# lucidrains/transfusion-pytorch

Measured on NVIDIA H100. Metric: train tokens/sec (text+latent) at d=512 L=8 seq=1024, higher is better.
Workload: dtype bf16

## Files before the change

include/tfx_b200.h:

```cpp
#ifndef TFX_B200_H
#define TFX_B200_H

#ifdef __cplusplus
extern "C" {
#endif

#define TFX_B200_VERSION 200

const char* tfx_last_error(void);
int tfx_version(void);
int tfx_init(int device);


int tfx_gemm_set_cluster_mode(int mode);

int tfx_gemm_store(const void* A, long long lda, int a_mn_major, const void* B, long long ldb, int b_mn_major, int M, int N, int K,
                   float* out_f32, long long ld_f32, void* out_bf16, long long ld_bf16, const float* bias, const long long* row_off,
                   float alpha, int accumulate, int k_splits, void* stream);

int tfx_gemm_qkvg(const void* u, long long ldu, const void* W, long long ldw, int M, int H, int D, void* q, void* k, void* v, float* gates, float* qk_inv,
                  const float* q_gamma, const float* k_gamma, const int* rope_pos, const float* rope_cs_t , int rope_len,
                  const int* kv_rows, float* mix_pre, void* stream);

int tfx_gemm_resid(const void* A, long long lda, const void* A2, long long lda2, int K1, const void* W, long long ldw, int M, int N, int K, const float* bias,
                   const float* x_res, float* x_out, void* x_out_bf16, void* y_bf16, const int* cond_row, const float* zgate, long long zgate_ld,
                   const float* layerscale, void* stream);

int tfx_gemm_geglu(const void* u, long long ldu, const void* W1p, long long ldw, const float* b1p, int M, int Np, int K, void* vg, void* h, void* stream);
int tfx_gemm_geglu_drop(const void* u, long long ldu, const void* W1p, long long ldw, const float* b1p, int M, int Np, int K, void* vg, void* h,
                        const void* drop_key , float p, int layer, void* stream);

int tfx_attn_fwd(const void* q, const void* k, const void* v, long long ld_q, long long ld_k, long long ld_v, const float* gates, int H,
                 const int* kv_limit, const int* tile_q0, const int* tile_qend, const int* tile_kv0, const int* tile_kvend, int n_tiles,
                 void* o, long long ld_o, float* lse, int M, float scale, float softcap, const float* skip_if_fast , void* stream);
int tfx_attn_fast_params(const float* q_gamma, const float* k_gamma, int dim_head, float scale, float softcap, float* params , void* stream);
int tfx_attn_fwd_tc(const void* q, const void* k, const void* v, long long ld_q, long long ld_k, long long ld_v, const float* gates, int H,
                    const int* kv_limit, const int* tile_q0, const int* tile_qend, const int* tile_kv0, const int* tile_kvend, int n_tiles,
                    void* o, long long ld_o, float* lse, int M, int M_kv , float scale, float softcap,
                    const float* fast_params, void* stream);
int tfx_attn_bwd_prep(const void* do_gated, const void* o_gated, const float* gates, void* do_pre, float* dsum_hm, float* dsum_mh, float* dq_zero, int M, int H, void* stream);
int tfx_attn_bwd(const void* q, const void* k, const void* v, const void* do_pre, long long ld_q, long long ld_k, long long ld_v, long long ld_do,
                 const float* lse, const float* dsum_hm, const int* kv_limit, const int* kt_kv0, const int* kt_kvend, const int* kt_q0, const int* kt_qend,
                 int n_kv_tiles, float* dq, float* dk, void* dv, long long ld_dv, int M, int H, float scale, float softcap, const float* skip_if_fast ,
                 void* stream);
int tfx_attn_bwd_tc(const void* q, const void* k, const void* v, const void* do_pre, long long ld_q, long long ld_k, long long ld_v, long long ld_do,
                    const float* lse, const float* dsum_hm, const int* kv_limit, const int* kt_kv0, const int* kt_kvend, const int* kt_q0, const int* kt_qend,
                    const int* kt_order ,
                    int n_kv_tiles, float* dq, float* dk, void* dv, long long ld_dv, int M, int H, float scale, float softcap, const float* fast_params, void* stream);
int tfx_qk_bwd_pack(const float* dq, const float* dk, const void* q_bf16, const void* k_bf16, const float* qk_inv, const float* q_gamma, const float* k_gamma,
                    const int* rope_pos, const float* rope_cs, const float* gates, const float* dsum_mh, void* dqkvg_bf16, long long out_ld,
                    float* dq_gamma, float* dk_gamma, int M, int H, void* stream);

int tfx_attn_residual_bwd2(const void* const* hiddens_bf16, int n_hiddens, int own, const float* const* gammas, const float* const* pseudo_queries,
                           const float* const* dx_later, const float* const* scalars_later, int n_later, const float* dx_out, const float* x_out, const float* lse,
                           float* grad_hidden, float* scalars_out, int scalar_stride, float* dgamma, float* dpseudo_query, float* workspace, int M, int D, void* stream);

int tfx_laser_v_fwd(const void* v, long long ld_v, const int* rows, void* v_laser, long long ld_vl, int M, int H, float clamp, void* stream);
int tfx_laser_out_fwd(const void* o_laser, const float* gates, void* att, int M, int H, void* stream);
int tfx_laser_bwd_prep(const void* d_att, const void* o_laser, const float* gates, void* do_pre, float* dsum_hm, float* dsum_mh, float* dq_zero, int M, int H, void* stream);
int tfx_laser_v_bwd(void* dv_inout, long long ld_dv, const void* v, long long ld_v, int M, int H, float clamp, void* stream);
int tfx_vmix_fwd(void* v_inout, long long ld_v, const int* rows, const void* v_first, long long ld_v0, const float* mix_pre, const float* mix_bias, int M, int H, void* stream);
int tfx_vmix_bwd(void* dv_inout, long long ld_dv, const void* v_mixed, long long ld_v, const void* v_first, long long ld_v0, const float* mix_pre, const float* mix_bias,
                 float* dv_first_acc, void* dmix_bf16, long long ld_dmix, int M, int H, void* stream);
int tfx_add_f32_into_bf16(void* dst_bf16, long long ld_dst, const float* src, long long ld_src, int M, int N, void* stream);

int tfx_adaln_fwd(const float* x, const int* cond_row, const float* film, long long film_ld, const float* ln_gamma,
                  void* u_bf16, float* stats, int M, int D, void* stream);
int tfx_adaln_bwd(const float* du, const float* x, const float* stats, const int* cond_row, const float* film, long long film_ld,
                  const float* ln_gamma, float* dx_accum, float* dfilm, long long dfilm_ld, float* dln_gamma, int M, int D, void* stream);
int tfx_resid_bwd(const float* dx, const void* y_bf16, const int* cond_row, const float* zgate, long long zgate_ld, const float* layerscale,
                  void* dy_bf16, float* dzgate, long long dzgate_ld, float* dlayerscale, float* dbias, int M, int D, void* stream);
int tfx_attn_residual_fwd(const float* const* hiddens, int n_hiddens, const float* gamma, const float* pseudo_query,
                          float* x_out, void* x_out_bf16, float* lse_out, int M, int D, void* stream);
long long tfx_attn_residual_bwd_workspace_floats(int M, int D);
int tfx_attn_residual_bwd(const float* const* hiddens, float* const* dhiddens, int n_hiddens, const float* gamma, const float* pseudo_query,
                          const float* dx_out, const float* x_out, const float* lse, float* dgamma, float* dpseudo_query, float* workspace, int M, int D,
                          int init , void* stream);
int tfx_attn_residual_fwd_h16(const void* const* hiddens_bf16, int n_hiddens, const float* gamma, const float* pseudo_query,
                              float* x_out, void* x_out_bf16, float* lse_out, int M, int D, void* stream);
int tfx_attn_residual_bwd_h16(const void* const* hiddens_bf16, float* const* dhiddens, int n_hiddens, const float* gamma, const float* pseudo_query,
                              const float* dx_out, const float* x_out, const float* lse, float* dgamma, float* dpseudo_query, float* workspace, int M, int D, int init,
                              void* stream);
int tfx_rmsnorm_fwd(const float* x, const float* gamma, float* out_f32, void* out_bf16, const int* slot, void* out_mod_bf16, int M, int D, void* stream);
int tfx_rmsnorm_bwd(const float* dout, const float* x, const float* gamma, float* dx, float* dgamma, int M, int D, void* stream);
int tfx_embed_assemble(const int* text_id, const float* emb, const float* modtok, const int* slot, float* x0, void* x0_bf16, int M, int D, void* stream);
int tfx_embed_bwd(const float* dx0, const int* text_id, const int* slot, float* demb, void* dmodtok_bf16, int M, int D, void* stream);
int tfx_clean_flow_fwd(const float* out, const int* row_token, const float* modtok, const float* cond_times, const int* cond_row, float eps, void* omod_bf16, int S, int D, void* stream);
int tfx_clean_flow_bwd(float* dmod_inout, float* dmodtok_neg, const int* row_token, const float* cond_times, const int* cond_row, float eps, int S, int D, void* stream);
int tfx_scatter_add_rows(float* dst, const float* src, const int* row_map, int S, int D, void* stream);

int tfx_flow_noise(const float* x, const float* eps, const float* t_row, void* noised_bf16, long long ld_noised, float* noised_f32, float* flow, long long S, int dl, void* stream);
int tfx_time_features(const float* times, const float* fourier_w, void* feats_bf16, int n, int half_dim, int ld, void* stream);
int tfx_table_op(const float* a, long long ld_a, const float* b, long long ld_b, float* out_f32, long long ld_of, void* out_bf16, long long ld_ob, long long rows, int cols,
                 int op, void* stream);
int tfx_geglu_bwd_rows_per_block(void);
int tfx_geglu_bwd(const void* dh_bf16, const void* vg_bf16, void* dvg_bf16, long long M, int inner_pad, const int* col_map, float* dbias, float* partials, void* stream);
int tfx_geglu_bwd_drop(const void* dh_bf16, const void* vg_bf16, void* dvg_bf16, long long M, int inner_pad, const int* col_map, float* dbias, float* partials,
                       const void* drop_key , float p, int layer, void* stream);
int tfx_ce_fwd_bwd(const float* logits, long long ld_logits, const int* labels, int V, int vlimit, float gscale, void* dlogits_bf16, long long ld_dlogits,
                   double* loss_sum, int* n_valid, int M, void* stream);
int tfx_mse_fwd_bwd(const float* pred, long long ld_pred, const float* flow, void* dpred_bf16, long long ld_dpred, float gscale, double* sumsq, long long S, int dl, void* stream);
int tfx_colsum_bf16(const void* in_bf16, long long ld, long long M, int N, const int* col_map, float* out, void* stream);
int tfx_colsum_f32(const float* in, long long ld, long long M, int N, const int* col_map , float* out, void* stream);
typedef struct TfxPackJob {
  const float* src; long long ld_src; const int* row_src ; void* dst ;
  long long R_dst; int C_src; int C_dst; int dst_f32; int pad_;
} TfxPackJob;
int tfx_cast_pack_multi(const TfxPackJob* jobs_dev, const int* blk_job_dev, const int* blk_first_dev, int n_blocks, void* stream);
int tfx_cast_bf16(const float* src, void* dst_bf16, long long n, void* stream);
int tfx_scale_bf16(void* p_bf16, const float* scale_ptr, long long n, void* stream);
int tfx_axpy_f32(float* y, const float* x, float a, long long n, void* stream);
int tfx_rope_table(const float* freqs, float* cos_sin, float* cos_sin_t, int max_pos, int n_freqs, void* stream);
int tfx_adam_step(float* params, float* grads, float* exp_avg, float* exp_avg_sq, long long n, float lr, float beta1, float beta2, float eps, float weight_decay,
                  int decoupled_wd, int step, float grad_scale, int zero_grads ,
                  int* step_dev ,
                  void* stream);

int tfx_grad_sumsq(const float* grads, long long n, double* sumsq_accum, void* stream);
int tfx_clip_by_norm(float* grads, long long n, const double* sumsq, float max_norm, float pre_scale, void* stream);
int tfx_ema_update(float* ema, const float* params, long long n, float decay, void* stream);


int tfx_decode_prep(const int* state, int S, int cap, int slab0, int* text_id, int* rope_pos, int* kv_row, int* kv_limit, int* tile_q0, int* tile_qend, int* tile_kv0,
                    int* tile_kvend, int* counters, void* stream);
int tfx_attn_decode(const void* q, const void* k, const void* v, long long ld_q, long long ld_k, long long ld_v, const float* gates, int H, const int* kv_limit,
                    const int* tile_q0, const int* tile_kv0, const int* tile_kvend, int n_tiles, void* o, long long ld_o, float scale, float softcap, void* stream);
int tfx_sample_tokens(const float* logits, long long ld_logits, const int* rows, int V, int vlimit, int* state, int S, int* hist, int hist_cap, int eos_id, const int* som_ids,
                      int n_som, int max_length, float temperature, float min_p, unsigned long long seed, int* counters, int advance, void* stream);
int tfx_ode_pre(const float* y, const float* f_prev, float* x_eval, long long n, int dup, const float* tab, const int* idx, float* cond_times, int n_cond, void* stream);
int tfx_ode_post(float* y, float* f_prev, const float* pred_cond, const float* pred_uncond, float cfg_scale, long long n, const float* tab, const int* idx, void* stream);
int tfx_counter_inc(int* counter, void* stream);

#ifdef __cplusplus
}
#endif
#endif
```

transfusion_pytorch_b200/_lib.py:

```python
from __future__ import annotations

import ctypes
import os
from ctypes import c_void_p, c_int, c_longlong, c_ulonglong, c_float, c_char_p, POINTER

_HERE = os.path.dirname(os.path.abspath(__file__))
LIB_PATH = os.path.join(_HERE, 'libtfx_b200.so')

_lib = None

VP, I, LL, F, ULL = c_void_p, c_int, c_longlong, c_float, c_ulonglong

SIGNATURES = {
    'tfx_init': [I],
    'tfx_gemm_set_cluster_mode': [I],
    'tfx_gemm_store': [VP, LL, I, VP, LL, I, I, I, I, VP, LL, VP, LL, VP, VP, F, I, I, VP],
    'tfx_gemm_qkvg': [VP, LL, VP, LL, I, I, I, VP, VP, VP, VP, VP, VP, VP, VP, VP, I, VP, VP, VP],
    'tfx_gemm_resid': [VP, LL, VP, LL, I, VP, LL, I, I, I, VP, VP, VP, VP, VP, VP, VP, LL, VP, VP],
    'tfx_gemm_geglu': [VP, LL, VP, LL, VP, I, I, I, VP, VP, VP],
    'tfx_gemm_geglu_drop': [VP, LL, VP, LL, VP, I, I, I, VP, VP, VP, F, I, VP],
    'tfx_attn_fwd': [VP, VP, VP, LL, LL, LL, VP, I, VP, VP, VP, VP, VP, I, VP, LL, VP, I, F, F, VP, VP],
    'tfx_attn_fwd_tc': [VP, VP, VP, LL, LL, LL, VP, I, VP, VP, VP, VP, VP, I, VP, LL, VP, I, I, F, F, VP, VP],
    'tfx_attn_fast_params': [VP, VP, I, F, F, VP, VP],
    'tfx_attn_bwd_prep': [VP, VP, VP, VP, VP, VP, VP, I, I, VP],
    'tfx_attn_bwd': [VP, VP, VP, VP, LL, LL, LL, LL, VP, VP, VP, VP, VP, VP, VP, I, VP, VP, VP, LL, I, I, F, F, VP, VP],
    'tfx_attn_bwd_tc': [VP, VP, VP, VP, LL, LL, LL, LL, VP, VP, VP, VP, VP, VP, VP, VP, I, VP, VP, VP, LL, I, I, F, F, VP, VP],
    'tfx_qk_bwd_pack': [VP, VP, VP, VP, VP, VP, VP, VP, VP, VP, VP, VP, LL, VP, VP, I, I, VP],
    'tfx_adaln_fwd': [VP, VP, VP, LL, VP, VP, VP, I, I, VP],
    'tfx_adaln_bwd': [VP, VP, VP, VP, VP, LL, VP, VP, VP, LL, VP, I, I, VP],
    'tfx_resid_bwd': [VP, VP, VP, VP, LL, VP, VP, VP, LL, VP, VP, I, I, VP],
    'tfx_attn_residual_fwd': [VP, I, VP, VP, VP, VP, VP, I, I, VP],
    'tfx_attn_residual_bwd': [VP, VP, I, VP, VP, VP, VP, VP, VP, VP, VP, I, I, I, VP],
    'tfx_attn_residual_bwd2': [VP, I, I, VP, VP, VP, VP, I, VP, VP, VP, VP, VP, I, VP, VP, VP, I, I, VP],
    'tfx_attn_residual_fwd_h16': [VP, I, VP, VP, VP, VP, VP, I, I, VP],
    'tfx_attn_residual_bwd_h16': [VP, VP, I, VP, VP, VP, VP, VP, VP, VP, VP, I, I, I, VP],
    'tfx_rmsnorm_fwd': [VP, VP, VP, VP, VP, VP, I, I, VP],
    'tfx_rmsnorm_bwd': [VP, VP, VP, VP, VP, I, I, VP],
    'tfx_embed_assemble': [VP, VP, VP, VP, VP, VP, I, I, VP],
    'tfx_embed_bwd': [VP, VP, VP, VP, VP, I, I, VP],
    'tfx_scatter_add_rows': [VP, VP, VP, I, I, VP],
    'tfx_flow_noise': [VP, VP, VP, VP, LL, VP, VP, LL, I, VP],
    'tfx_time_features': [VP, VP, VP, I, I, I, VP],
    'tfx_table_op': [VP, LL, VP, LL, VP, LL, VP, LL, LL, I, I, VP],
    'tfx_geglu_bwd': [VP, VP, VP, LL, I, VP, VP, VP, VP],
    'tfx_geglu_bwd_drop': [VP, VP, VP, LL, I, VP, VP, VP, VP, F, I, VP],
    'tfx_ce_fwd_bwd': [VP, LL, VP, I, I, F, VP, LL, VP, VP, I, VP],
    'tfx_mse_fwd_bwd': [VP, LL, VP, VP, LL, F, VP, LL, I, VP],
    'tfx_colsum_bf16': [VP, LL, LL, I, VP, VP, VP],
    'tfx_colsum_f32': [VP, LL, LL, I, VP, VP, VP],
    'tfx_cast_pack_multi': [VP, VP, VP, I, VP],
    'tfx_cast_bf16': [VP, VP, LL, VP],
    'tfx_scale_bf16': [VP, VP, LL, VP],
    'tfx_axpy_f32': [VP, VP, F, LL, VP],
    'tfx_rope_table': [VP, VP, VP, I, I, VP],
    'tfx_grad_sumsq': [VP, LL, VP, VP],
    'tfx_clip_by_norm': [VP, LL, VP, F, F, VP],
    'tfx_ema_update': [VP, VP, LL, F, VP],
    'tfx_adam_step': [VP, VP, VP, VP, LL, F, F, F, F, F, I, I, F, I, VP, VP],
    'tfx_decode_prep': [VP, I, I, I, VP, VP, VP, VP, VP, VP, VP, VP, VP, VP],
    'tfx_attn_decode': [VP, VP, VP, LL, LL, LL, VP, I, VP, VP, VP, VP, I, VP, LL, F, F, VP],
    'tfx_sample_tokens': [VP, LL, VP, I, I, VP, I, VP, I, I, VP, I, I, F, F, ULL, VP, I, VP],
    'tfx_ode_pre': [VP, VP, VP, LL, I, VP, VP, VP, I, VP],
    'tfx_ode_post': [VP, VP, VP, VP, F, LL, VP, VP, VP],
    'tfx_counter_inc': [VP, VP],
    'tfx_clean_flow_fwd': [VP, VP, VP, VP, VP, F, VP, I, I, VP],
    'tfx_clean_flow_bwd': [VP, VP, VP, VP, VP, F, I, I, VP],
    'tfx_laser_v_fwd': [VP, LL, VP, VP, LL, I, I, F, VP],
    'tfx_laser_out_fwd': [VP, VP, VP, I, I, VP],
    'tfx_laser_bwd_prep': [VP, VP, VP, VP, VP, VP, VP, I, I, VP],
    'tfx_laser_v_bwd': [VP, LL, VP, LL, I, I, F, VP],
    'tfx_vmix_fwd': [VP, LL, VP, VP, LL, VP, VP, I, I, VP],
    'tfx_vmix_bwd': [VP, LL, VP, LL, VP, LL, VP, VP, VP, VP, LL, I, I, VP],
    'tfx_add_f32_into_bf16': [VP, LL, VP, LL, I, I, VP],
}

EXPORTED = ['tfx_last_error', 'tfx_version', 'tfx_geglu_bwd_rows_per_block', 'tfx_attn_residual_bwd_workspace_floats'] + list(SIGNATURES)


class TfxError(RuntimeError):
    pass


def library_present() -> bool:
    return os.path.isfile(LIB_PATH)


def load():
    global _lib
    if _lib is not None:
        return _lib
    if not library_present():
        raise TfxError(
            f'{LIB_PATH} is missing: the sm_90a CUDA extension has not been built. '
            'Run `python -c "import __graft_entry__ as g; g.build()"` (or `make -C transfusion_pytorch_b200/csrc`). '
            'There is no CPU / eager fallback.')
    lib = ctypes.CDLL(LIB_PATH)
    lib.tfx_last_error.restype = c_char_p
    lib.tfx_last_error.argtypes = []
    lib.tfx_version.restype = c_int
    lib.tfx_version.argtypes = []
    lib.tfx_geglu_bwd_rows_per_block.restype = c_int
    lib.tfx_geglu_bwd_rows_per_block.argtypes = []
    lib.tfx_attn_residual_bwd_workspace_floats.restype = c_longlong
    lib.tfx_attn_residual_bwd_workspace_floats.argtypes = [c_int, c_int]
    for name, argtypes in SIGNATURES.items():
        fn = getattr(lib, name)
        fn.argtypes = argtypes
        fn.restype = c_int
    _lib = lib
    return lib


def check(rc: int, name: str):
    if rc != 0:
        msg = _lib.tfx_last_error().decode(errors = 'replace') if _lib is not None else ''
        raise TfxError(f'{name} failed (code {rc}): {msg}')


class Ops:

    def __init__(self):
        self.lib = load()
        import torch
        self._torch = torch
        self.launches = 0
        self.timing = None
        self.order = None

    def stream(self):
        return self._torch.cuda.current_stream().cuda_stream

    def __getattr__(self, name):
        fn = getattr(self.lib, 'tfx_' + name)
        torch = self._torch

        def call(*args):
            conv = []
            for a in args:
                if a is None:
                    conv.append(None)
                elif torch.is_tensor(a):
                    conv.append(a.data_ptr())
                else:
                    conv.append(a)
            self.launches += 1
            if self.timing is not None:
                e0, e1 = torch.cuda.Event(enable_timing = True), torch.cuda.Event(enable_timing = True)
                e0.record()
                rc = fn(*conv, self.stream())
                e1.record()
                self.timing.setdefault(name, []).append((e0, e1, args))
                if self.order is not None:
                    self.order.append(name)
            else:
                rc = fn(*conv, self.stream())
            if rc != 0:
                check(rc, 'tfx_' + name)
        call.__name__ = name
        setattr(self, name, call)
        return call
```

transfusion_pytorch_b200/csrc/attention_sm90.cu:

```cuda
#include "sm90_ptx.cuh"
#include "common.cuh"
#include "gemm_sm90.cuh"
#include "../../include/tfx_b200.h"

namespace tfx {

int num_sms();

constexpr int FA_BM = 128, FA_BN = 128;
constexpr int FA_THREADS = 256;
constexpr int FA_SMEM = 16384 * 5 + 1024  + 256 ;
constexpr float FA_YMAX = 0.75f;

#define FA_C0 9.9999722832e-01f
#define FA_C1 -3.3323076483e-01f
#define FA_C2 1.3226091649e-01f
#define FA_C3 -4.9280448379e-02f
#define FA_C4 1.2318833231e-02f

__global__ void attn_fast_params_k(const float* __restrict__ gq, const float* __restrict__ gk, int n, float scale, float cap, float* __restrict__ params) {
  const int lane = threadIdx.x;
  float a = 0.f, b = 0.f;
  for (int i = lane; i < n; i += 32) { a = fmaxf(a, fabsf(gq[i] + 1.f)); b = fmaxf(b, fabsf(gk[i] + 1.f)); }
  a = warp_max(a); b = warp_max(b);
  if (lane == 0) {
    const float xmax = 1.01f * (float)n * a * b * scale;
    const float ymax = xmax / cap;
    params[0] = (ymax <= FA_YMAX && isfinite(ymax)) ? 1.f : 0.f;
    params[1] = xmax;
  }
}

__device__ __forceinline__ float ex2_approx(float x) { float y; asm("ex2.approx.ftz.f32 %0, %1;" : "=f"(y) : "f"(x)); return y; }

struct FaPoly {
  float a0, a1, a2, a3, a4;
  __device__ __forceinline__ FaPoly(float scale, float cap) {
    const float k1 = scale / cap, KL = cap * 1.4426950408889634f, k2 = k1 * k1;
    a0 = KL * k1 * FA_C0; a1 = KL * k1 * k2 * FA_C1; a2 = KL * k1 * k2 * k2 * FA_C2; a3 = KL * k1 * k2 * k2 * k2 * FA_C3; a4 = KL * k1 * k2 * k2 * k2 * k2 * FA_C4;
  }
  __device__ __forceinline__ float operator()(float x) const { return x * tail(x); }
  __device__ __forceinline__ float minus(float x, float m) const { return fmaf(x, tail(x), -m); }
  __device__ __forceinline__ float tail(float x) const {
    const float X = x * x;
    float g = fmaf(a4, X, a3);
    g = fmaf(g, X, a2);
    g = fmaf(g, X, a1);
    return fmaf(g, X, a0);
  }
};

template <bool MASKED>
__device__ __forceinline__ void fwd_p(const float (&s)[64], uint32_t (&pf)[8][4], float& l_a, float& l_b, int key0, int lim_a, int lim_b,
                                      const FaPoly& poly, float m2, int t) {
#pragma unroll
  for (int n8 = 0; n8 < 16; ++n8) {
    const int key = key0 + n8 * 8 + 2 * t;
    float p0 = ex2_approx(poly.minus(s[4 * n8], m2)), p1 = ex2_approx(poly.minus(s[4 * n8 + 1], m2));
    float p2 = ex2_approx(poly.minus(s[4 * n8 + 2], m2)), p3 = ex2_approx(poly.minus(s[4 * n8 + 3], m2));
    if (MASKED) {
      p0 = key <= lim_a ? p0 : 0.f; p1 = key + 1 <= lim_a ? p1 : 0.f;
      p2 = key <= lim_b ? p2 : 0.f; p3 = key + 1 <= lim_b ? p3 : 0.f;
    }
    l_a += p0 + p1; l_b += p2 + p3;
    pf[n8 >> 1][(n8 & 1) * 2] = pack_bf16(p0, p1);
    pf[n8 >> 1][(n8 & 1) * 2 + 1] = pack_bf16(p2, p3);
  }
}

__global__ void __launch_bounds__(FA_THREADS, 2)
attn_fwd_tc_k(const __grid_constant__ CUtensorMap tmQ, const __grid_constant__ CUtensorMap tmK, const __grid_constant__ CUtensorMap tmV,
              const float* __restrict__ gates, int H, const int* __restrict__ kv_limit, const int* __restrict__ tile_q0, const int* __restrict__ tile_qend,
              const int* __restrict__ tile_kv0, const int* __restrict__ tile_kvend, __nv_bfloat16* __restrict__ o, long long ld_o, float* __restrict__ lse,
              int M, float scale, float cap, const float* __restrict__ fast) {
  if (fast[0] == 0.f) return;
  extern __shared__ uint8_t fa_smem_raw[];
  uint8_t* smem = reinterpret_cast<uint8_t*>((reinterpret_cast<uintptr_t>(fa_smem_raw) + 1023) & ~uintptr_t(1023));
  uint8_t* sQ = smem;
  uint8_t* sK = smem + 16384;
  uint8_t* sV = smem + 49152;
  uint64_t* bars = reinterpret_cast<uint64_t*>(smem + 81920);
  uint64_t *q_full = bars, *kv_full = bars + 1;

  const int tile = gridDim.x - 1 - blockIdx.x;
  const int head = blockIdx.y;
  const int tid = threadIdx.x, warp = tid >> 5, lane = tid & 31;
  const int cwg = warp >> 2, w4 = warp & 3, g = lane >> 2, t = lane & 3;
  const int q0 = tile_q0[tile], q_end = tile_qend[tile], kv0 = tile_kv0[tile], kv_end = tile_kvend[tile];
  const int n_kv = (kv_end - kv0 + FA_BN - 1) / FA_BN;

  if (tid == 0) {
    tma_prefetch_desc(&tmQ); tma_prefetch_desc(&tmK); tma_prefetch_desc(&tmV);
    mbar_init(q_full, 1); mbar_init(&kv_full[0], 1); mbar_init(&kv_full[1], 1);
    mbar_fence_init();
  }
  __syncthreads();
  if (tid == 0) {
    mbar_expect_tx(q_full, 16384);
    tma_load_2d(&tmQ, q_full, sQ, head * 64, q0);
    for (int j = 0; j < 2 && j < n_kv; ++j) {
      mbar_expect_tx(&kv_full[j], 32768);
      tma_load_2d(&tmK, &kv_full[j], sK + j * 16384, head * 64, kv0 + j * FA_BN);
      tma_load_2d(&tmV, &kv_full[j], sV + j * 16384, head * 64, kv0 + j * FA_BN);
    }
  }

  const int row_a = q0 + cwg * 64 + w4 * 16 + g, row_b = row_a + 8;
  const int lim_a = row_a < q_end ? kv_limit[row_a] : -1;
  const int lim_b = row_b < q_end ? kv_limit[row_b] : -1;
  const FaPoly poly(scale, cap);
  const float m2 = fast[1] * 1.4426950408889634f;
  float oacc[32];
#pragma unroll
  for (int i = 0; i < 32; ++i) oacc[i] = 0.f;
  float l_a = 0.f, l_b = 0.f;
  const uint32_t aQ = smem_u32(sQ) + cwg * 8192;
  mbar_wait(q_full, 0);

  for (int j = 0; j < n_kv; ++j) {
    const int b = j & 1;
    mbar_wait(&kv_full[b], (j >> 1) & 1);
    const uint32_t aK = smem_u32(sK + b * 16384), aV = smem_u32(sV + b * 16384);
    float s[64];
    wgmma_fence();
#pragma unroll
    for (int k = 0; k < 4; ++k) wgmma_m64n128_ss<0, 0>(s, wgmma_desc_sw128(aQ + k * 32, 16, 1024), wgmma_desc_sw128(aK + k * 32, 16, 1024), k > 0 ? 1u : 0u);
    wgmma_commit();
    wgmma_wait<0>();
    wgmma_reg_fence(s);
    const int key0 = kv0 + j * FA_BN;
    uint32_t pf[8][4];
    if (__all_sync(0xffffffffu, key0 + FA_BN - 1 <= min(lim_a, lim_b))) fwd_p<false>(s, pf, l_a, l_b, key0, lim_a, lim_b, poly, m2, t);
    else fwd_p<true>(s, pf, l_a, l_b, key0, lim_a, lim_b, poly, m2, t);
    wgmma_reg_fence(oacc);
    wgmma_fence();
#pragma unroll
    for (int kk = 0; kk < 8; ++kk) wgmma_m64n64_rs<1>(oacc, pf[kk], wgmma_desc_sw128(aV + kk * 2048, 8192, 1024), 1u);
    wgmma_commit();
    wgmma_wait<0>();
    wgmma_reg_fence(oacc);
    __syncthreads();
    if (tid == 0 && j + 2 < n_kv) {
      mbar_expect_tx(&kv_full[b], 32768);
      tma_load_2d(&tmK, &kv_full[b], sK + b * 16384, head * 64, kv0 + (j + 2) * FA_BN);
      tma_load_2d(&tmV, &kv_full[b], sV + b * 16384, head * 64, kv0 + (j + 2) * FA_BN);
    }
  }
  l_a += __shfl_xor_sync(0xffffffffu, l_a, 1); l_a += __shfl_xor_sync(0xffffffffu, l_a, 2);
  l_b += __shfl_xor_sync(0xffffffffu, l_b, 1); l_b += __shfl_xor_sync(0xffffffffu, l_b, 2);
  float ga = l_a > 0.f ? 1.f / l_a : 0.f, gb = l_b > 0.f ? 1.f / l_b : 0.f;
  if (gates) {
    if (row_a < q_end) ga *= 1.f / (1.f + __expf(-gates[(long long)row_a * H + head]));
    if (row_b < q_end) gb *= 1.f / (1.f + __expf(-gates[(long long)row_b * H + head]));
  }
  if (row_a < q_end) {
    __nv_bfloat16* dst = o + (long long)row_a * ld_o + head * 64 + 2 * t;
#pragma unroll
    for (int n8 = 0; n8 < 8; ++n8) *reinterpret_cast<uint32_t*>(dst + n8 * 8) = pack_bf16(oacc[4 * n8] * ga, oacc[4 * n8 + 1] * ga);
    if (t == 0 && lse) lse[(long long)head * M + row_a] = fast[1] + logf(l_a);
  }
  if (row_b < q_end) {
    __nv_bfloat16* dst = o + (long long)row_b * ld_o + head * 64 + 2 * t;
#pragma unroll
    for (int n8 = 0; n8 < 8; ++n8) *reinterpret_cast<uint32_t*>(dst + n8 * 8) = pack_bf16(oacc[4 * n8 + 2] * gb, oacc[4 * n8 + 3] * gb);
    if (t == 0 && lse) lse[(long long)head * M + row_b] = fast[1] + logf(l_b);
  }
}


constexpr int FB_BQ = 64;
constexpr int FB_THREADS = 256;
constexpr int FB_STAGES = 4;
constexpr int FB_STAGE = 16384;
constexpr int FB_RING = 32768;
constexpr int FB_ROW_BOX = FB_BQ + 4;
constexpr int FB_ROW_SLOT = 384, FB_ROWS_STAGE = 3 * FB_ROW_SLOT;
constexpr int FB_ROWS = FB_RING + FB_STAGES * FB_STAGE;
constexpr int FB_DS = FB_ROWS + ((FB_STAGES * FB_ROWS_STAGE + 1023) & ~1023);
constexpr int FB_DQ = FB_DS + 2 * 16384;
constexpr int FB_BAR = FB_DQ + 2 * 16384;
constexpr int FB_SMEM = FB_BAR + 256 + 1024 ;
constexpr int FB_BAR_DS_FULL = 1, FB_BAR_DS_EMPTY = 3, FB_BAR_DQ = 5;

template <bool MASKED>
__device__ __forceinline__ void bwd_p(float (&sacc)[32], uint32_t (&pf)[4][4], const int* sLim, const float* sLse, int key_a, int key_b, int qvalid,
                                      const FaPoly& poly, float oms_c, float scale, int t) {
#pragma unroll
  for (int n8 = 0; n8 < 8; ++n8) {
    const int c0 = n8 * 8 + 2 * t;
    const float lse2[2] = {sLse[c0] * 1.4426950408889634f, sLse[c0 + 1] * 1.4426950408889634f};
    int lim[2] = {0, 0};
    if (MASKED) {
      lim[0] = c0 < qvalid ? sLim[c0] : -1;
      lim[1] = c0 + 1 < qvalid ? sLim[c0 + 1] : -1;
    }
    float pv[4];
#pragma unroll
    for (int r = 0; r < 2; ++r)
#pragma unroll
      for (int c = 0; c < 2; ++c) {
        const int e = 4 * n8 + 2 * r + c;
        const float e2 = poly(sacc[e]);
        float p = ex2_approx(e2 - lse2[c]);
        if (MASKED) p = ((r == 0 ? key_a : key_b) <= lim[c]) ? p : 0.f;
        pv[2 * r + c] = p;
        sacc[e] = p * fmaf(e2 * e2, oms_c, scale);
      }
    pf[n8 >> 1][(n8 & 1) * 2] = pack_bf16(pv[0], pv[1]);
    pf[n8 >> 1][(n8 & 1) * 2 + 1] = pack_bf16(pv[2], pv[3]);
  }
}

__global__ void __launch_bounds__(FB_THREADS, 1)
attn_bwd_tc_k(const __grid_constant__ CUtensorMap tmQ, const __grid_constant__ CUtensorMap tmK, const __grid_constant__ CUtensorMap tmV,
              const __grid_constant__ CUtensorMap tmDO, const __grid_constant__ CUtensorMap tmLim, const __grid_constant__ CUtensorMap tmLse,
              const __grid_constant__ CUtensorMap tmD, const __grid_constant__ CUtensorMap tmDQ,
              const int* __restrict__ kt_kv0, const int* __restrict__ kt_kvend, const int* __restrict__ kt_q0, const int* __restrict__ kt_qend,
              const int* __restrict__ kt_order, float* __restrict__ dk, __nv_bfloat16* __restrict__ dv, long long ld_dv, int M, int H, float scale, float cap,
              const float* __restrict__ fast) {
  if (fast[0] == 0.f) return;
  extern __shared__ uint8_t fb_smem_raw[];
  uint8_t* smem = reinterpret_cast<uint8_t*>((reinterpret_cast<uintptr_t>(fb_smem_raw) + 1023) & ~uintptr_t(1023));
  uint8_t* sK = smem;
  uint8_t* sV = smem + 16384;
  uint8_t* sDS = smem + FB_DS;
  uint64_t* bars = reinterpret_cast<uint64_t*>(smem + FB_BAR);
  uint64_t *full = bars, *empty = bars + FB_STAGES, *kv_full = bars + 2 * FB_STAGES;

  const int idx = blockIdx.x;
  const int tt = idx / H;
  const int tile = kt_order ? kt_order[tt] : tt;
  const int head = idx - tt * H;
  const int kv0 = kt_kv0[tile], kv_end = kt_kvend[tile], q_begin = kt_q0[tile], q_end = kt_qend[tile];
  const int n_q = (q_end - q_begin + FB_BQ - 1) / FB_BQ;
  const int tid = threadIdx.x, warp = tid >> 5, lane = tid & 31;

  if (tid == 0) {
    tma_prefetch_desc(&tmQ); tma_prefetch_desc(&tmK); tma_prefetch_desc(&tmV); tma_prefetch_desc(&tmDO);
    for (int s = 0; s < FB_STAGES; ++s) { mbar_init(&full[s], 1); mbar_init(&empty[s], 8); }
    mbar_init(kv_full, 1);
    mbar_fence_init();
  }
  __syncthreads();

  auto load_step = [&](int j) {
    const int sl = j % FB_STAGES;
    const int qb = q_begin + j * FB_BQ;
    uint8_t* st = smem + FB_RING + sl * FB_STAGE;
    uint8_t* rows = smem + FB_ROWS + sl * FB_ROWS_STAGE;
    mbar_expect_tx(&full[sl], FB_STAGE + 3 * FB_ROW_BOX * 4);
    tma_load_2d(&tmQ, &full[sl], st, head * 64, qb);
    tma_load_2d(&tmDO, &full[sl], st + 8192, head * 64, qb);
    tma_load_1d(&tmLim, &full[sl], rows, qb & ~3);
    tma_load_1d(&tmLse, &full[sl], rows + FB_ROW_SLOT, (head * M + qb) & ~3);
    tma_load_1d(&tmD, &full[sl], rows + 2 * FB_ROW_SLOT, (head * M + qb) & ~3);
  };
  if (tid == 0) {
    mbar_expect_tx(kv_full, 32768);
    tma_load_2d(&tmK, kv_full, sK, head * 64, kv0);
    tma_load_2d(&tmV, kv_full, sV, head * 64, kv0);
    for (int j = 0; j < FB_STAGES && j < n_q; ++j) load_step(j);
  }
  const int cwg = warp >> 2, w4 = warp & 3, g = lane >> 2, t = lane & 3;
  const bool leader = (tid & 127) == 0;
  const FaPoly poly(scale, cap);
  const float KL = cap * 1.4426950408889634f;
  const float oms_c = -scale / (KL * KL);
  const int key_a = kv0 + cwg * 64 + w4 * 16 + g, key_b = key_a + 8;
  const int warp_key_last = kv0 + cwg * 64 + w4 * 16 + 15;
  float dvacc[32], dkacc[32];
#pragma unroll
  for (int i = 0; i < 32; ++i) { dvacc[i] = 0.f; dkacc[i] = 0.f; }
  const uint32_t aK = smem_u32(sK) + cwg * 8192, aV = smem_u32(sV) + cwg * 8192, aKall = smem_u32(sK);
  const int ds_row0 = cwg * 64 + w4 * 16 + g;
  uint8_t* sDQ = smem + FB_DQ + cwg * 16384;
  mbar_wait(kv_full, 0);

  int s = 0; uint32_t phase = 0;
  for (int i = 0; i < n_q; ++i) {
    const int b = i & 1;
    const int qb = q_begin + i * FB_BQ;
    mbar_wait(&full[s], phase);
    const uint32_t aQ = smem_u32(smem + FB_RING + s * FB_STAGE), aDO = aQ + 8192;
    const int* sLim = reinterpret_cast<const int*>(smem + FB_ROWS + s * FB_ROWS_STAGE) + (qb & 3);
    const float* sLse = reinterpret_cast<const float*>(smem + FB_ROWS + s * FB_ROWS_STAGE + FB_ROW_SLOT) + ((head * M + qb) & 3);
    const float* sD = reinterpret_cast<const float*>(smem + FB_ROWS + s * FB_ROWS_STAGE + 2 * FB_ROW_SLOT) + ((head * M + qb) & 3);
    float sacc[32], pacc[32];
    wgmma_fence();
#pragma unroll
    for (int k = 0; k < 4; ++k) wgmma_m64n64_ss<0, 0>(sacc, wgmma_desc_sw128(aK + k * 32, 16, 1024), wgmma_desc_sw128(aQ + k * 32, 16, 1024), k > 0 ? 1u : 0u);
    wgmma_commit();
#pragma unroll
    for (int k = 0; k < 4; ++k) wgmma_m64n64_ss<0, 0>(pacc, wgmma_desc_sw128(aV + k * 32, 16, 1024), wgmma_desc_sw128(aDO + k * 32, 16, 1024), k > 0 ? 1u : 0u);
    wgmma_commit();
    if (tid == 0 && i >= 2 && i - 2 + FB_STAGES < n_q) {
      mbar_wait(&empty[(i - 2) % FB_STAGES], ((i - 2) / FB_STAGES) & 1);
      load_step(i - 2 + FB_STAGES);
    }
    const int qvalid = q_end - qb;
    const bool full_vis = qvalid >= FB_BQ && warp_key_last <= __reduce_min_sync(0xffffffffu, min(sLim[lane], sLim[lane + 32]));
    wgmma_wait<1>();
    wgmma_reg_fence(sacc);
    uint32_t pf[4][4], dsf[4][4];
    if (full_vis) bwd_p<false>(sacc, pf, sLim, sLse, key_a, key_b, qvalid, poly, oms_c, scale, t);
    else bwd_p<true>(sacc, pf, sLim, sLse, key_a, key_b, qvalid, poly, oms_c, scale, t);
    wgmma_wait<0>();
    wgmma_reg_fence(pacc);
#pragma unroll
    for (int n8 = 0; n8 < 8; ++n8) {
      const float d0 = sD[n8 * 8 + 2 * t], d1 = sD[n8 * 8 + 2 * t + 1];
      dsf[n8 >> 1][(n8 & 1) * 2] = pack_bf16(sacc[4 * n8] * (pacc[4 * n8] - d0), sacc[4 * n8 + 1] * (pacc[4 * n8 + 1] - d1));
      dsf[n8 >> 1][(n8 & 1) * 2 + 1] = pack_bf16(sacc[4 * n8 + 2] * (pacc[4 * n8 + 2] - d0), sacc[4 * n8 + 3] * (pacc[4 * n8 + 3] - d1));
    }
    uint8_t* dsb = sDS + b * 16384;
    if (cwg != b && i >= 2) named_bar_sync(FB_BAR_DS_EMPTY + b, 256);
#pragma unroll
    for (int n8 = 0; n8 < 8; ++n8) {
      const int r0 = ds_row0, r1 = ds_row0 + 8;
      *reinterpret_cast<uint32_t*>(dsb + r0 * 128 + ((n8 ^ (r0 & 7)) << 4) + t * 4) = dsf[n8 >> 1][(n8 & 1) * 2];
      *reinterpret_cast<uint32_t*>(dsb + r1 * 128 + ((n8 ^ (r1 & 7)) << 4) + t * 4) = dsf[n8 >> 1][(n8 & 1) * 2 + 1];
    }
    fence_proxy_async_smem();
    if (cwg == b) named_bar_sync(FB_BAR_DS_FULL + b, 256);
    else named_bar_arrive(FB_BAR_DS_FULL + b, 256);
    wgmma_reg_fence(dvacc);
    wgmma_reg_fence(dkacc);
    wgmma_fence();
#pragma unroll
    for (int kk = 0; kk < 4; ++kk) wgmma_m64n64_rs<1>(dvacc, pf[kk], wgmma_desc_sw128(aDO + kk * 2048, 8192, 1024), 1u);
#pragma unroll
    for (int kk = 0; kk < 4; ++kk) wgmma_m64n64_rs<1>(dkacc, dsf[kk], wgmma_desc_sw128(aQ + kk * 2048, 8192, 1024), 1u);
    wgmma_commit();
    if (cwg == b) {
      float qacc[32];
      const uint32_t aDS = smem_u32(dsb);
      wgmma_fence();
#pragma unroll
      for (int kk = 0; kk < 8; ++kk) wgmma_m64n64_ss<1, 1>(qacc, wgmma_desc_sw128(aDS + kk * 2048, 8192, 1024), wgmma_desc_sw128(aKall + kk * 2048, 8192, 1024), kk > 0 ? 1u : 0u);
      wgmma_commit();
      wgmma_wait<0>();
      wgmma_reg_fence(dvacc);
      wgmma_reg_fence(dkacc);
      wgmma_reg_fence(qacc);
      __syncwarp();
      if (lane == 0) mbar_arrive(&empty[s]);
      if (i + 2 < n_q) named_bar_arrive(FB_BAR_DS_EMPTY + b, 256);
      if (leader) bulk_wait_read_all();
      named_bar_sync(FB_BAR_DQ + cwg, 128);
      const int r0 = w4 * 16 + g, r1 = r0 + 8;
#pragma unroll
      for (int n8 = 0; n8 < 8; ++n8) {
        const int chunk = 2 * (n8 & 3) + (t >> 1), off = (n8 >> 2) * 8192 + (t & 1) * 8;
        *reinterpret_cast<float2*>(sDQ + off + r0 * 128 + ((chunk ^ (r0 & 7)) << 4)) = make_float2(qacc[4 * n8], qacc[4 * n8 + 1]);
        *reinterpret_cast<float2*>(sDQ + off + r1 * 128 + ((chunk ^ (r1 & 7)) << 4)) = make_float2(qacc[4 * n8 + 2], qacc[4 * n8 + 3]);
      }
      fence_proxy_async_smem();
      named_bar_sync(FB_BAR_DQ + cwg, 128);
      if (leader) {
        tma_reduce_add_2d(&tmDQ, sDQ, head * 64, qb);
        tma_reduce_add_2d(&tmDQ, sDQ + 8192, head * 64 + 32, qb);
        bulk_commit();
      }
    } else {
      wgmma_wait<0>();
      wgmma_reg_fence(dvacc);
      wgmma_reg_fence(dkacc);
      __syncwarp();
      if (lane == 0) mbar_arrive(&empty[s]);
    }
    if (++s == FB_STAGES) { s = 0; phase ^= 1; }
  }
  if (leader) bulk_wait_all();
#pragma unroll
  for (int n8 = 0; n8 < 8; ++n8) {
    if (key_a < kv_end) {
      *reinterpret_cast<float2*>(dk + (long long)key_a * H * 64 + head * 64 + n8 * 8 + 2 * t) = make_float2(dkacc[4 * n8], dkacc[4 * n8 + 1]);
      *reinterpret_cast<uint32_t*>(dv + (long long)key_a * ld_dv + head * 64 + n8 * 8 + 2 * t) = pack_bf16(dvacc[4 * n8], dvacc[4 * n8 + 1]);
    }
    if (key_b < kv_end) {
      *reinterpret_cast<float2*>(dk + (long long)key_b * H * 64 + head * 64 + n8 * 8 + 2 * t) = make_float2(dkacc[4 * n8 + 2], dkacc[4 * n8 + 3]);
      *reinterpret_cast<uint32_t*>(dv + (long long)key_b * ld_dv + head * 64 + n8 * 8 + 2 * t) = pack_bf16(dvacc[4 * n8 + 2], dvacc[4 * n8 + 3]);
    }
  }
}

inline int make_tmap_rows(CUtensorMap* tm, CUtensorMapDataType type, const void* ptr, long long n) {
  PFN_encodeTiled enc = get_encode_fn();
  if (!enc) return -1;
  cuuint64_t dims[1] = {(cuuint64_t)n};
  cuuint64_t strides[1] = {0};
  cuuint32_t box[1] = {FB_ROW_BOX}, estr[1] = {1};
  CUresult r = enc(tm, type, 1, const_cast<void*>(ptr), dims, strides, box, estr, CU_TENSOR_MAP_INTERLEAVE_NONE, CU_TENSOR_MAP_SWIZZLE_NONE,
                   CU_TENSOR_MAP_L2_PROMOTION_NONE, CU_TENSOR_MAP_FLOAT_OOB_FILL_NONE);
  return r == CUDA_SUCCESS ? 0 : -(int)r - 1000;
}

inline int make_tmap_dq(CUtensorMap* tm, float* dq, int M, int H) {
  PFN_encodeTiled enc = get_encode_fn();
  if (!enc) return -1;
  cuuint64_t dims[2] = {(cuuint64_t)H * 64, (cuuint64_t)M};
  cuuint64_t strides[1] = {(cuuint64_t)H * 64 * 4};
  cuuint32_t box[2] = {32, FB_BQ}, estr[2] = {1, 1};
  CUresult r = enc(tm, CU_TENSOR_MAP_DATA_TYPE_FLOAT32, 2, dq, dims, strides, box, estr, CU_TENSOR_MAP_INTERLEAVE_NONE, CU_TENSOR_MAP_SWIZZLE_128B,
                   CU_TENSOR_MAP_L2_PROMOTION_L2_256B, CU_TENSOR_MAP_FLOAT_OOB_FILL_NONE);
  return r == CUDA_SUCCESS ? 0 : -(int)r - 1000;
}

}

using namespace tfx;
#define ST(s) reinterpret_cast<cudaStream_t>(s)

extern "C" {

int tfx_attn_fast_params(const float* q_gamma, const float* k_gamma, int dim_head, float scale, float softcap, float* params, void* stream) {
  TFX_REQUIRE(dim_head > 0 && softcap > 0.f, "attn_fast_params: bad arguments");
  attn_fast_params_k<<<1, 32, 0, ST(stream)>>>(q_gamma, k_gamma, dim_head, scale, softcap, params);
  return check_launch("attn_fast_params");
}

int tfx_attn_fwd_tc(const void* q, const void* k, const void* v, long long ld_q, long long ld_k, long long ld_v, const float* gates, int H,
                    const int* kv_limit, const int* tile_q0, const int* tile_qend, const int* tile_kv0, const int* tile_kvend, int n_tiles,
                    void* o, long long ld_o, float* lse, int M, int M_kv, float scale, float softcap, const float* fast_params, void* stream) {
  if (n_tiles <= 0) return 0;
  if (M_kv <= 0) M_kv = M;
  TFX_REQUIRE(fast_params != nullptr, "attn_fwd_tc: fast_params (from tfx_attn_fast_params) is required");
  TFX_REQUIRE(ld_q % 8 == 0 && ld_k % 8 == 0 && ld_v % 8 == 0 && ld_o % 8 == 0, "attn_fwd_tc: row pitches must be multiples of 8 bf16");
  CUtensorMap tq, tk, tv;
  int rc;
  if ((rc = make_tmap_bf16(&tq, q, (long long)H * 64, M, ld_q, FA_BM)) || (rc = make_tmap_bf16(&tk, k, (long long)H * 64, M_kv, ld_k, FA_BN)) ||
      (rc = make_tmap_bf16(&tv, v, (long long)H * 64, M_kv, ld_v, FA_BN))) {
    set_error("attn_fwd_tc: cuTensorMapEncodeTiled failed (%d)", rc);
    return rc;
  }
  static bool attr_set = false;
  if (!attr_set) {
    if (cudaFuncSetAttribute(attn_fwd_tc_k, cudaFuncAttributeMaxDynamicSharedMemorySize, FA_SMEM) != cudaSuccess) { set_error("attn_fwd_tc: cannot raise dynamic smem"); return -2; }
    attr_set = true;
  }
  attn_fwd_tc_k<<<dim3(n_tiles, H), FA_THREADS, FA_SMEM, ST(stream)>>>(tq, tk, tv, gates, H, kv_limit, tile_q0, tile_qend, tile_kv0, tile_kvend, (__nv_bfloat16*)o, ld_o, lse, M,
                                                                      scale, softcap, fast_params);
  return check_launch("attn_fwd_tc");
}

int tfx_attn_bwd_tc(const void* q, const void* k, const void* v, const void* do_pre, long long ld_q, long long ld_k, long long ld_v, long long ld_do,
                    const float* lse, const float* dsum_hm, const int* kv_limit, const int* kt_kv0, const int* kt_kvend, const int* kt_q0, const int* kt_qend,
                    const int* kt_order, int n_kv_tiles, float* dq, float* dk, void* dv, long long ld_dv, int M, int H, float scale, float softcap, const float* fast_params,
                    void* stream) {
  if (n_kv_tiles <= 0) return 0;
  TFX_REQUIRE(fast_params != nullptr, "attn_bwd_tc: fast_params (from tfx_attn_fast_params) is required");
  TFX_REQUIRE(ld_q % 8 == 0 && ld_k % 8 == 0 && ld_v % 8 == 0 && ld_do % 8 == 0 && ld_dv % 8 == 0, "attn_bwd_tc: row pitches must be multiples of 8 bf16");
  CUtensorMap tq, tk, tv, tdo, tlim, tlse, td, tdq;
  int rc;
  if ((rc = make_tmap_bf16(&tq, q, (long long)H * 64, M, ld_q, FB_BQ)) || (rc = make_tmap_bf16(&tk, k, (long long)H * 64, M, ld_k, FA_BN)) ||
      (rc = make_tmap_bf16(&tv, v, (long long)H * 64, M, ld_v, FA_BN)) || (rc = make_tmap_bf16(&tdo, do_pre, (long long)H * 64, M, ld_do, FB_BQ)) ||
      (rc = make_tmap_rows(&tlim, CU_TENSOR_MAP_DATA_TYPE_INT32, kv_limit, M)) || (rc = make_tmap_rows(&tlse, CU_TENSOR_MAP_DATA_TYPE_FLOAT32, lse, (long long)H * M)) ||
      (rc = make_tmap_rows(&td, CU_TENSOR_MAP_DATA_TYPE_FLOAT32, dsum_hm, (long long)H * M)) || (rc = make_tmap_dq(&tdq, dq, M, H))) {
    set_error("attn_bwd_tc: cuTensorMapEncodeTiled failed (%d): kv_limit, lse, dsum and dq must be 16-byte aligned", rc);
    return rc;
  }
  static bool attr_set = false;
  if (!attr_set) {
    if (cudaFuncSetAttribute(attn_bwd_tc_k, cudaFuncAttributeMaxDynamicSharedMemorySize, FB_SMEM) != cudaSuccess) { set_error("attn_bwd_tc: cannot raise dynamic smem"); return -2; }
    attr_set = true;
  }
  attn_bwd_tc_k<<<n_kv_tiles * H, FB_THREADS, FB_SMEM, ST(stream)>>>(tq, tk, tv, tdo, tlim, tlse, td, tdq, kt_kv0, kt_kvend, kt_q0, kt_qend, kt_order, dk,
                                                                     (__nv_bfloat16*)dv, ld_dv, M, H, scale, softcap, fast_params);
  return check_launch("attn_bwd_tc");
}

}
```

transfusion_pytorch_b200/csrc/sm90_ptx.cuh:

```cuda
#pragma once
#include <cuda.h>
#include <cuda_runtime.h>
#include <cuda_bf16.h>
#include <stdint.h>
#include <stdio.h>

namespace tfx {

#ifndef TFX_SPIN_LIMIT
#define TFX_SPIN_LIMIT (1u << 24)
#endif

__device__ __forceinline__ uint32_t smem_u32(const void* p) {
  return static_cast<uint32_t>(__cvta_generic_to_shared(p));
}

__device__ __forceinline__ void mbar_init(uint64_t* bar, uint32_t count) {
  asm volatile("mbarrier.init.shared::cta.b64 [%0], %1;" ::"r"(smem_u32(bar)), "r"(count));
}
__device__ __forceinline__ void mbar_fence_init() {
  asm volatile("fence.mbarrier_init.release.cluster;" ::: "memory");
}
__device__ __forceinline__ void mbar_expect_tx(uint64_t* bar, uint32_t bytes) {
  asm volatile("mbarrier.arrive.expect_tx.shared::cta.b64 _, [%0], %1;" ::"r"(smem_u32(bar)), "r"(bytes) : "memory");
}
__device__ __forceinline__ void mbar_arrive(uint64_t* bar) {
  asm volatile("mbarrier.arrive.shared::cta.b64 _, [%0];" ::"r"(smem_u32(bar)) : "memory");
}
__device__ __forceinline__ bool mbar_try_wait(uint64_t* bar, uint32_t parity) {
  uint32_t ok;
  asm volatile(
      "{\n\t.reg .pred p;\n\t"
      "mbarrier.try_wait.parity.shared::cta.b64 p, [%1], %2;\n\t"
      "selp.u32 %0, 1, 0, p;\n\t}"
      : "=r"(ok) : "r"(smem_u32(bar)), "r"(parity) : "memory");
  return ok != 0;
}
__device__ __forceinline__ void mbar_wait(uint64_t* bar, uint32_t parity) {
  uint32_t spins = 0;
  while (!mbar_try_wait(bar, parity)) {
    if (++spins > TFX_SPIN_LIMIT) {
#if defined(TFX_DEBUG_SPIN) && TFX_DEBUG_SPIN
      printf("tfx: mbarrier timeout block %d thread %d bar %u parity %u\n", blockIdx.x, threadIdx.x, smem_u32(bar), parity);
#endif
      __trap();
    }
  }
}

__device__ __forceinline__ void tma_prefetch_desc(const CUtensorMap* m) {
  asm volatile("prefetch.tensormap [%0];" ::"l"(reinterpret_cast<uint64_t>(m)) : "memory");
}
__device__ __forceinline__ void tma_load_2d(const CUtensorMap* m, uint64_t* bar, void* smem, int c0, int c1) {
  asm volatile(
      "cp.async.bulk.tensor.2d.shared::cluster.global.mbarrier::complete_tx::bytes [%0], [%1, {%3, %4}], [%2];"
      ::"r"(smem_u32(smem)), "l"(reinterpret_cast<uint64_t>(m)), "r"(smem_u32(bar)), "r"(c0), "r"(c1)
      : "memory");
}
__device__ __forceinline__ void tma_load_1d(const CUtensorMap* m, uint64_t* bar, void* smem, int c0) {
  asm volatile(
      "cp.async.bulk.tensor.1d.shared::cluster.global.mbarrier::complete_tx::bytes [%0], [%1, {%3}], [%2];"
      ::"r"(smem_u32(smem)), "l"(reinterpret_cast<uint64_t>(m)), "r"(smem_u32(bar)), "r"(c0)
      : "memory");
}
__device__ __forceinline__ void tma_reduce_add_2d(const CUtensorMap* m, const void* smem, int c0, int c1) {
  asm volatile("cp.reduce.async.bulk.tensor.2d.global.shared::cta.add.tile.bulk_group [%0, {%2, %3}], [%1];"
               ::"l"(reinterpret_cast<uint64_t>(m)), "r"(smem_u32(smem)), "r"(c0), "r"(c1) : "memory");
}
__device__ __forceinline__ void bulk_commit() { asm volatile("cp.async.bulk.commit_group;" ::: "memory"); }
__device__ __forceinline__ void bulk_wait_read_all() { asm volatile("cp.async.bulk.wait_group.read 0;" ::: "memory"); }
__device__ __forceinline__ void bulk_wait_all() { asm volatile("cp.async.bulk.wait_group 0;" ::: "memory"); }
__device__ __forceinline__ void tma_load_2d_multicast(const CUtensorMap* m, uint64_t* bar, void* smem, int c0, int c1, uint16_t mask) {
  asm volatile(
      "cp.async.bulk.tensor.2d.shared::cluster.global.mbarrier::complete_tx::bytes.multicast::cluster [%0], [%1, {%3, %4}], [%2], %5;"
      ::"r"(smem_u32(smem)), "l"(reinterpret_cast<uint64_t>(m)), "r"(smem_u32(bar)), "r"(c0), "r"(c1), "h"(mask)
      : "memory");
}
__device__ __forceinline__ uint32_t cluster_ctarank() { uint32_t r; asm volatile("mov.u32 %0, %%cluster_ctarank;" : "=r"(r)); return r; }
__device__ __forceinline__ void cluster_sync_all() {
  asm volatile("barrier.cluster.arrive.release.aligned;\n\tbarrier.cluster.wait.acquire.aligned;" ::: "memory");
}
__device__ __forceinline__ void mbar_arrive_cluster(uint64_t* bar, uint32_t rank) {
  uint32_t remote;
  asm volatile("mapa.shared::cluster.u32 %0, %1, %2;" : "=r"(remote) : "r"(smem_u32(bar)), "r"(rank));
  asm volatile("mbarrier.arrive.release.cluster.shared::cluster.b64 _, [%0];" ::"r"(remote) : "memory");
}
__device__ __forceinline__ void fence_proxy_async_smem() {
  asm volatile("fence.proxy.async.shared::cta;" ::: "memory");
}
__device__ __forceinline__ void named_bar_sync(int id, int count) {
  asm volatile("bar.sync %0, %1;" ::"r"(id), "r"(count) : "memory");
}
__device__ __forceinline__ void named_bar_arrive(int id, int count) {
  asm volatile("bar.arrive %0, %1;" ::"r"(id), "r"(count) : "memory");
}

template <int N> __device__ __forceinline__ void setmaxnreg_dec() { asm volatile("setmaxnreg.dec.sync.aligned.u32 %0;" ::"n"(N)); }
template <int N> __device__ __forceinline__ void setmaxnreg_inc() { asm volatile("setmaxnreg.inc.sync.aligned.u32 %0;" ::"n"(N)); }

__device__ __forceinline__ void wgmma_fence() { asm volatile("wgmma.fence.sync.aligned;" ::: "memory"); }
__device__ __forceinline__ void wgmma_commit() { asm volatile("wgmma.commit_group.sync.aligned;" ::: "memory"); }
template <int N> __device__ __forceinline__ void wgmma_wait() { asm volatile("wgmma.wait_group.sync.aligned %0;" ::"n"(N) : "memory"); }
template <int N> __device__ __forceinline__ void wgmma_reg_fence(float (&d)[N]) {
#pragma unroll
  for (int i = 0; i < N; ++i) asm volatile("" : "+f"(d[i])::"memory");
}

template <int TA, int TB>
__device__ __forceinline__ void wgmma_m64n128_ss(float (&d)[64], uint64_t da, uint64_t db, uint32_t accumulate) {
  asm volatile(
      "{\n\t.reg .pred p;\n\t"
      "setp.ne.b32 p, %66, 0;\n\t"
      "wgmma.mma_async.sync.aligned.m64n128k16.f32.bf16.bf16 "
      "{%0, %1, %2, %3, %4, %5, %6, %7, %8, %9, %10, %11, %12, %13, %14, %15, %16, %17, %18, %19, %20, %21, %22, %23, %24, %25, %26, %27, %28, %29, %30, %31, %32, %33, %34, %35, %36, %37, %38, %39, %40, %41, %42, %43, %44, %45, %46, %47, %48, %49, %50, %51, %52, %53, %54, %55, %56, %57, %58, %59, %60, %61, %62, %63}, "
      "%64, %65, p, 1, 1, %67, %68;\n\t}"
      : "+f"(d[0]), "+f"(d[1]), "+f"(d[2]), "+f"(d[3]), "+f"(d[4]), "+f"(d[5]), "+f"(d[6]), "+f"(d[7]), "+f"(d[8]), "+f"(d[9]), "+f"(d[10]), "+f"(d[11]), "+f"(d[12]), "+f"(d[13]), "+f"(d[14]), "+f"(d[15]), "+f"(d[16]), "+f"(d[17]), "+f"(d[18]), "+f"(d[19]), "+f"(d[20]), "+f"(d[21]), "+f"(d[22]), "+f"(d[23]), "+f"(d[24]), "+f"(d[25]), "+f"(d[26]), "+f"(d[27]), "+f"(d[28]), "+f"(d[29]), "+f"(d[30]), "+f"(d[31]), "+f"(d[32]), "+f"(d[33]), "+f"(d[34]), "+f"(d[35]), "+f"(d[36]), "+f"(d[37]), "+f"(d[38]), "+f"(d[39]), "+f"(d[40]), "+f"(d[41]), "+f"(d[42]), "+f"(d[43]), "+f"(d[44]), "+f"(d[45]), "+f"(d[46]), "+f"(d[47]), "+f"(d[48]), "+f"(d[49]), "+f"(d[50]), "+f"(d[51]), "+f"(d[52]), "+f"(d[53]), "+f"(d[54]), "+f"(d[55]), "+f"(d[56]), "+f"(d[57]), "+f"(d[58]), "+f"(d[59]), "+f"(d[60]), "+f"(d[61]), "+f"(d[62]), "+f"(d[63])
      : "l"(da), "l"(db), "r"(accumulate), "n"(TA), "n"(TB));
}
template <int TA, int TB>
__device__ __forceinline__ void wgmma_m64n64_ss(float (&d)[32], uint64_t da, uint64_t db, uint32_t accumulate) {
  asm volatile(
      "{\n\t.reg .pred p;\n\t"
      "setp.ne.b32 p, %34, 0;\n\t"
      "wgmma.mma_async.sync.aligned.m64n64k16.f32.bf16.bf16 "
      "{%0, %1, %2, %3, %4, %5, %6, %7, %8, %9, %10, %11, %12, %13, %14, %15, %16, %17, %18, %19, %20, %21, %22, %23, %24, %25, %26, %27, %28, %29, %30, %31}, "
      "%32, %33, p, 1, 1, %35, %36;\n\t}"
      : "+f"(d[0]), "+f"(d[1]), "+f"(d[2]), "+f"(d[3]), "+f"(d[4]), "+f"(d[5]), "+f"(d[6]), "+f"(d[7]), "+f"(d[8]), "+f"(d[9]), "+f"(d[10]), "+f"(d[11]), "+f"(d[12]), "+f"(d[13]), "+f"(d[14]), "+f"(d[15]), "+f"(d[16]), "+f"(d[17]), "+f"(d[18]), "+f"(d[19]), "+f"(d[20]), "+f"(d[21]), "+f"(d[22]), "+f"(d[23]), "+f"(d[24]), "+f"(d[25]), "+f"(d[26]), "+f"(d[27]), "+f"(d[28]), "+f"(d[29]), "+f"(d[30]), "+f"(d[31])
      : "l"(da), "l"(db), "r"(accumulate), "n"(TA), "n"(TB));
}
template <int TB>
__device__ __forceinline__ void wgmma_m64n64_rs(float (&d)[32], const uint32_t (&a)[4], uint64_t db, uint32_t accumulate) {
  asm volatile(
      "{\n\t.reg .pred p;\n\t"
      "setp.ne.b32 p, %37, 0;\n\t"
      "wgmma.mma_async.sync.aligned.m64n64k16.f32.bf16.bf16 "
      "{%0, %1, %2, %3, %4, %5, %6, %7, %8, %9, %10, %11, %12, %13, %14, %15, %16, %17, %18, %19, %20, %21, %22, %23, %24, %25, %26, %27, %28, %29, %30, %31}, "
      "{%32, %33, %34, %35}, %36, p, 1, 1, %38;\n\t}"
      : "+f"(d[0]), "+f"(d[1]), "+f"(d[2]), "+f"(d[3]), "+f"(d[4]), "+f"(d[5]), "+f"(d[6]), "+f"(d[7]), "+f"(d[8]), "+f"(d[9]), "+f"(d[10]), "+f"(d[11]), "+f"(d[12]), "+f"(d[13]), "+f"(d[14]), "+f"(d[15]), "+f"(d[16]), "+f"(d[17]), "+f"(d[18]), "+f"(d[19]), "+f"(d[20]), "+f"(d[21]), "+f"(d[22]), "+f"(d[23]), "+f"(d[24]), "+f"(d[25]), "+f"(d[26]), "+f"(d[27]), "+f"(d[28]), "+f"(d[29]), "+f"(d[30]), "+f"(d[31])
      : "r"(a[0]), "r"(a[1]), "r"(a[2]), "r"(a[3]), "l"(db), "r"(accumulate), "n"(TB));
}

__device__ __forceinline__ uint64_t wgmma_desc_sw128(uint32_t smem_addr, uint32_t lbo_bytes, uint32_t sbo_bytes) {
  uint64_t d = 0;
  d |= (uint64_t)((smem_addr >> 4) & 0x3FFF);
  d |= (uint64_t)((lbo_bytes >> 4) & 0x3FFF) << 16;
  d |= (uint64_t)((sbo_bytes >> 4) & 0x3FFF) << 32;
  d |= (uint64_t)1 << 62;
  return d;
}

}
```

transfusion_pytorch_b200/engine.py:

```python
from __future__ import annotations

import math
import os
import ctypes
from dataclasses import dataclass

import numpy as np
import torch
from torch import Tensor

from . import _lib
from ._pinned import POOL
from .modality_processing import RaggedBatch

BF16, F32, I32, I64 = torch.bfloat16, torch.float32, torch.int32, torch.int64


def _round_up(x: int, m: int) -> int:
    return (x + m - 1) // m * m


_EMPTY_I32 = np.zeros(0, dtype = np.int32)


def posemb_tables(params, lens, device):
    out = []
    for (w0, b0, w2, b2), L in zip(params, lens):
        seq = torch.arange(int(L), device = device, dtype = F32)[:, None]
        pre = seq * w0.reshape(1, -1) + b0
        act = pre * torch.sigmoid(pre)
        out.append((seq, pre, act, act @ w2.t() + b2))
    return out


def posemb_add(rows: Tensor, tables, coords):
    for (_, _, _, e), c in zip(tables, coords):
        rows += e.index_select(0, c)


def posemb_backward(d_rows: Tensor, tables, coords, params, grads):
    for (seq, pre, act, e), c, (w0, b0, w2, b2), (gw0, gb0, gw2, gb2) in zip(tables, coords, params, grads):
        d_e = torch.zeros_like(e).index_add_(0, c, d_rows)
        gw2 += d_e.t() @ act
        gb2 += d_e.sum(0)
        sig = torch.sigmoid(pre)
        d_pre = (d_e @ w2) * (sig * (1. + pre * (1. - sig)))
        gw0 += (d_pre * seq).sum(0)[:, None]
        gb0 += d_pre.sum(0)


class KVCache:

    def __init__(self, engine, n_slabs: int, cap: int):
        self.n_slabs, self.cap, self.rows = int(n_slabs), int(cap), int(n_slabs) * int(cap)
        nbytes = 2 * engine.depth * self.rows * engine.HI * 2
        assert nbytes < 96 << 30, f'kv cache of {nbytes / 2**30:.1f} GiB requested ({n_slabs} slabs x {cap} rows): lower max_length / batch the prompts'
        self.k = torch.zeros(engine.depth, self.rows, engine.HI, device = engine.device, dtype = BF16)
        self.v = torch.zeros(engine.depth, self.rows, engine.HI, device = engine.device, dtype = BF16)
        self.vl = torch.zeros_like(self.v) if engine.laser else None

    def slab_start(self, s):
        return np.asarray(s, dtype = np.int64) * self.cap


class Engine:
    def __init__(self, model):
        self.ops = _lib.Ops()
        self.model = model
        tr = model.transformer
        self.D, self.H, self.depth = tr.dim, tr.heads, tr.depth
        self.HI = self.H * 64
        self.inner = tr.ff_inner
        self.Ip = _round_up(self.inner, 64)
        self.NQ = 3 * self.HI + 128
        self.V = model.text_embed.weight.shape[0]
        self.Vp = _round_up(self.V, 8)
        self.Kt = _round_up(self.D + 1, 64)
        self.W = 2 * self.depth
        self.softcap = tr.softcap_value
        self.laser, self.laser_clamp, self.vres = tr.attn_laser, tr.laser_softclamp_value, tr.use_value_residual
        self.clean, self.clean_eps = bool(getattr(model, 'model_output_clean', False)), float(getattr(model, 'eps', 1e-2))
        self.posemb = tuple(bool(a) for a in getattr(model, 'add_pos_emb', ()))
        self.scale = 64 ** -0.5
        self.dls = list(model.dim_latents)
        self.dlp = [_round_up(d, 8) for d in self.dls]
        assert self.D % 128 == 0 and self.D <= 1024, 'model dim must be a multiple of 128 and <= 1024 for the row kernels'
        assert self.H % 2 == 0 and 2 <= self.H <= 32, 'heads must be even (two 64-wide heads per 128-column GEMM tile)'
        self.device = None
        self.flat = None
        self.ws = {}
        self._dirty = True
        self._ptr_arrays = []
        self.launches = 0
        self.graph_pins = None
        self.hid_bf16 = os.environ.get('TFX_HIDDEN_BF16', '1') == '1'
        self.ares_deferred = self.hid_bf16 and os.environ.get('TFX_ARES_DEFERRED', '1') == '1'
        self.frozen = False

    def _trainable(self):
        m = self.model
        skip = set()
        for mod in list(m.modality_encoder) + list(m.modality_decoder):
            if mod is not None:
                skip |= {id(p) for p in mod.parameters()}
        return [(n, p) for n, p in m.named_parameters() if p.requires_grad and id(p) not in skip]

    def attach(self):
        named = self._trainable()
        late = lambda n: ('.to_film.' in n) or ('.to_ada_ln_zero.' in n) or n.startswith('transformer.to_time_cond.')
        named = [(n, p) for n, p in named if not late(n)] + [(n, p) for n, p in named if late(n)]
        dev = named[0][1].device
        if dev.type != 'cuda':
            raise _lib.TfxError(f'the CUDA engine needs the model on a CUDA device (got {dev}); there is no CPU path')
        rc = self.ops.lib.tfx_init(dev.index if dev.index is not None else torch.cuda.current_device())
        _lib.check(rc, 'tfx_init')
        self.device = dev
        offs, total = {}, 0
        for n, p in named:
            offs[n] = total
            total += _round_up(p.numel(), 4)
        flat = torch.zeros(total, device = dev, dtype = F32)
        gflat = torch.zeros(total, device = dev, dtype = F32)
        for n, p in named:
            o, k = offs[n], p.numel()
            flat[o:o + k].copy_(p.data.reshape(-1).float())
            p.data = flat[o:o + k].view(p.shape)
            p.grad = gflat[o:o + k].view(p.shape)
        self.flat, self.gflat, self.offs, self.named = flat, gflat, offs, dict(named)
        self.named_first = named[0][1]
        self.exp_avg = self.exp_avg_sq = None
        self.opt_step = 0
        self._first_ptr = named[0][1].data_ptr()
        self.late_start = min((offs[n] for n, _ in named if late(n)), default = total)
        self._build_maps()
        self._dirty = True
        if not getattr(self, '_hooked', False):
            self.model.register_load_state_dict_post_hook(lambda *a, **k: self.mark_dirty())
            self._hooked = True

    def mark_dirty(self):
        self._dirty = True

    def ensure_attached(self):
        if self.flat is None or self.named_first.data_ptr() != self._first_ptr:
            self.attach()

    def P(self, name):
        return self.named[name]

    def _posemb_params(self, t, nax, grads = False):
        get = self.G if grads else self.P
        return [tuple(get(f'pos_emb_mlp.{t}.mlps.{a}.{k}') for k in ('0.weight', '0.bias', '2.weight', '2.bias')) for a in range(nax)]

    def G(self, name):
        o, p = self.offs[name], self.named[name]
        return self.gflat[o:o + p.numel()].view(p.shape)

    def _build_maps(self):
        dev, D, HI, H, inner, Ip = self.device, self.D, self.HI, self.H, self.inner, self.Ip
        src = np.full(2 * Ip, -1, dtype = np.int64)
        for t in range(Ip // 64):
            for j in range(64):
                c = 64 * t + j
                if c < inner:
                    src[128 * t + j] = c
                    src[128 * t + 64 + j] = inner + c
        self.w1_row_src = torch.from_numpy(src.astype(np.int32)).to(dev)
        self.w1_row_src64 = torch.from_numpy(src).to(dev)
        self.layer_maps = []
        for i in range(self.depth):
            pre = f'transformer.layers.{i}'
            w1_off = self.offs[f'{pre}.2.fn.net.0.weight']
            b1_off = self.offs[f'{pre}.2.fn.net.0.bias']
            w1_rows = torch.where(self.w1_row_src64 >= 0, w1_off + self.w1_row_src64 * D, torch.full_like(self.w1_row_src64, -1))
            b1_cols = torch.where(self.w1_row_src64 >= 0, b1_off + self.w1_row_src64, torch.full_like(self.w1_row_src64, -1)).to(I32)
            q_off, v_off, g_off = self.offs[f'{pre}.1.fn.to_qk.0.weight'], self.offs[f'{pre}.1.fn.to_v.0.weight'], self.offs[f'{pre}.1.fn.to_gates.0.weight']
            r = np.full(self.NQ, -1, dtype = np.int64)
            r[:2 * HI] = q_off + np.arange(2 * HI) * D
            r[2 * HI:3 * HI] = v_off + np.arange(HI) * D
            r[3 * HI:3 * HI + H] = g_off + np.arange(H) * D
            if f'{pre}.1.fn.to_learned_value_residual.0.weight' in self.offs:
                r[3 * HI + H:3 * HI + 2 * H] = self.offs[f'{pre}.1.fn.to_learned_value_residual.0.weight'] + np.arange(H) * D
            w2_off = self.offs[f'{pre}.2.fn.net.3.weight']
            w2_rows = torch.from_numpy(w2_off + np.arange(D, dtype = np.int64) * inner).to(dev)
            self.layer_maps.append(dict(w1_rows = w1_rows.contiguous(), b1_cols = b1_cols.contiguous(), qkvg_rows = torch.from_numpy(r).to(dev), w2_rows = w2_rows))
        rows = np.full(self.W * 3 * D, -1, dtype = np.int64)
        bias_idx = np.zeros(self.W * 3 * D, dtype = np.int64)
        for w in range(self.W):
            i, j = divmod(w, 2)
            pre = f'transformer.layers.{i}.{j + 1}'
            fo, zo = self.offs[f'{pre}.to_film.weight'], self.offs[f'{pre}.to_ada_ln_zero.weight']
            rows[w * 3 * D: w * 3 * D + 2 * D] = fo + np.arange(2 * D) * 4 * D
            rows[w * 3 * D + 2 * D: (w + 1) * 3 * D] = zo + np.arange(D) * 4 * D
            bias_idx[w * 3 * D: w * 3 * D + 2 * D] = self.offs[f'{pre}.to_film.bias'] + np.arange(2 * D)
            bias_idx[w * 3 * D + 2 * D: (w + 1) * 3 * D] = self.offs[f'{pre}.to_ada_ln_zero.bias'] + np.arange(D)
        self.fz_rows = torch.from_numpy(rows).to(dev)
        self.fz_bias_idx = torch.from_numpy(bias_idx).to(dev)
        tw = self.offs['transformer.to_time_cond.1.weight']
        self.wt_rows = torch.from_numpy(tw + np.arange(4 * D, dtype = np.int64) * (D + 1)).to(dev)

    def buf(self, name, shape, dtype, zero = False):
        t = self.ws.get(name)
        n = int(np.prod(shape)) if len(shape) else 1
        if t is None or t.dtype != dtype or t.numel() < n:
            if t is not None and self.graph_pins is not None:
                self.graph_pins.append(t)
            t = torch.empty(max(n, 1), device = self.device, dtype = dtype)
            self.ws[name] = t
            if zero:
                t.zero_()
        return t[:n].view(shape)

    def pin_workspaces(self):
        if self.graph_pins is None:
            self.graph_pins = []

    def _build_pack_jobs(self):
        D, HI, H, Ip, inner = self.D, self.HI, self.H, self.Ip, self.inner
        pk = self.packed = {}
        jobs = []
        def dst(name, rows, cols, dtype = BF16):
            t = pk[name] = torch.zeros(rows, cols, device = self.device, dtype = dtype) if cols else torch.zeros(rows, device = self.device, dtype = dtype)
            return t
        def job(src, ld_src, c_src, row_src, d, r_dst, c_dst):
            jobs.append((src, ld_src, c_src, row_src, d, r_dst, c_dst, 1 if d.dtype == F32 else 0))
        for i in range(self.depth):
            pre = f'transformer.layers.{i}'
            wq = dst(f'qkvg{i}', self.NQ, D)
            job(self.P(f'{pre}.1.fn.to_qk.0.weight'), D, D, None, wq, 2 * HI, D)
            job(self.P(f'{pre}.1.fn.to_v.0.weight'), D, D, None, wq[2 * HI:], HI, D)
            job(self.P(f'{pre}.1.fn.to_gates.0.weight'), D, D, None, wq[3 * HI:], H, D)
            if f'{pre}.1.fn.to_learned_value_residual.0.weight' in self.named:
                job(self.P(f'{pre}.1.fn.to_learned_value_residual.0.weight'), D, D, None, wq[3 * HI + H:], H, D)
            job(self.P(f'{pre}.1.fn.to_out.1.weight'), HI, HI, None, dst(f'wo{i}', D, HI), D, HI)
            job(self.P(f'{pre}.2.fn.net.0.weight'), D, D, self.w1_row_src, dst(f'w1{i}', 2 * Ip, D), 2 * Ip, D)
            job(self.P(f'{pre}.2.fn.net.3.weight'), inner, inner, None, dst(f'w2{i}', D, Ip), D, Ip)
            job(self.P(f'{pre}.2.fn.net.0.bias'), 1, 1, self.w1_row_src, dst(f'b1{i}', 2 * Ip, 0, F32), 2 * Ip, 1)
            if f'{pre}.0.weight' in self.named:
                job(self.P(f'{pre}.0.weight'), 2 * D, 2 * D, None, dst(f'wskip{i}', D, 2 * D), D, 2 * D)
        job(self.P('to_text_logits.weight'), D, D, None, dst('wvocab', self.V, D), self.V, D)
        for t, (dl, dlp) in enumerate(zip(self.dls, self.dlp)):
            job(self.P(f'model_to_latent_projs.{t}.weight'), D, D, None, dst(f'wm2l{t}', dl, D), dl, D)
            if f'latent_to_model_projs.{t}.weight' in self.named:
                job(self.P(f'latent_to_model_projs.{t}.weight'), dl, dl, None, dst(f'wl2m{t}', D, dlp), D, dlp)
        job(self.P('transformer.to_time_cond.1.weight'), D + 1, D + 1, None, dst('wt', 4 * D, self.Kt), 4 * D, self.Kt)
        wfz = dst('wfz', self.W * 3 * D, 4 * D)
        bfz = dst('bfz', self.W * 3 * D, 0, F32)
        for w in range(self.W):
            i, j = divmod(w, 2)
            pre = f'transformer.layers.{i}.{j + 1}'
            job(self.P(f'{pre}.to_film.weight'), 4 * D, 4 * D, None, wfz[w * 3 * D:], 2 * D, 4 * D)
            job(self.P(f'{pre}.to_ada_ln_zero.weight'), 4 * D, 4 * D, None, wfz[w * 3 * D + 2 * D:], D, 4 * D)
            job(self.P(f'{pre}.to_film.bias'), 2 * D, 2 * D, None, bfz[w * 3 * D:], 1, 2 * D)
            job(self.P(f'{pre}.to_ada_ln_zero.bias'), D, D, None, bfz[w * 3 * D + 2 * D:], 1, D)
        dt = np.dtype([('src', '<u8'), ('ld_src', '<i8'), ('row_src', '<u8'), ('dst', '<u8'), ('R_dst', '<i8'), ('C_src', '<i4'), ('C_dst', '<i4'),
                       ('dst_f32', '<i4'), ('pad', '<i4')])
        assert dt.itemsize == 56
        tab = np.zeros(len(jobs), dtype = dt)
        blk_job, blk_first = [], []
        for j, (src, ld_src, c_src, row_src, d, r_dst, c_dst, f32) in enumerate(jobs):
            tab[j] = (src.data_ptr(), ld_src, row_src.data_ptr() if row_src is not None else 0, d.data_ptr(), r_dst, c_src, c_dst, f32, 0)
            nb = (r_dst * c_dst + 2047) // 2048
            blk_first.append(len(blk_job))
            blk_job.extend([j] * nb)
        self._pack_tab = torch.from_numpy(tab.view(np.uint8).copy()).to(self.device)
        self._pack_blk_job = torch.tensor(blk_job, dtype = I32, device = self.device)
        self._pack_blk_first = torch.tensor(blk_first, dtype = I32, device = self.device)
        self._pack_nblocks = len(blk_job)
        self._pack_ptr = self._first_ptr

    def pack_weights(self, force = False):
        have = getattr(self, 'packed', None) is not None and getattr(self, '_pack_ptr', None) == self._first_ptr
        if have and not self._dirty and (self.frozen or not force):
            return
        if getattr(self, '_pack_ptr', None) != self._first_ptr:
            self._build_pack_jobs()
        self.ops.cast_pack_multi(self._pack_tab, self._pack_blk_job, self._pack_blk_first, self._pack_nblocks)
        if getattr(self, 'fastp', None) is None or self.fastp.device != self.device:
            self.fastp = torch.zeros(self.depth, 8, device = self.device, dtype = F32)
        for i in range(self.depth):
            pre = f'transformer.layers.{i}.1.fn'
            self.ops.attn_fast_params(self.P(f'{pre}.q_norm.gamma'), self.P(f'{pre}.k_norm.gamma'), 64, self.scale, self.softcap, self.fastp[i])
        self._dirty = False

    META_NAMES = ['text_id', 'label', 'kv_limit', 'rope_pos', 'cond_row', 'slot', 'tile_q0', 'tile_qend', 'tile_kv0', 'tile_kvend',
                  'kt_kv0', 'kt_kvend', 'kt_q0', 'kt_qend', 'row_token', 't2_q0', 't2_qend', 't2_kv0', 't2_kvend', 'k2_kv0', 'k2_kvend', 'k2_q0', 'k2_qend', 'k2_order', 'kv_row', 'pos_c0', 'pos_c1', 'pos_c2']

    def stage_meta(self, rb: RaggedBatch):
        ints = [getattr(rb, n) if getattr(rb, n) is not None else _EMPTY_I32 for n in self.META_NAMES]
        sizes = [_round_up(a.shape[0], 4) for a in ints]
        fl = np.concatenate([rb.cond_times, rb.row_time]).astype(np.float32)
        n_int, n_fl = sum(sizes), _round_up(fl.shape[0], 4)
        raw = POOL.take((n_int + n_fl) * 4)
        host = raw[:(n_int + n_fl) * 4].view(I32)
        hv = host.numpy()
        off = 0
        for a, s in zip(ints, sizes):
            hv[off:off + a.shape[0]] = a; off += s
        hv[n_int:n_int + fl.shape[0]] = fl.view(np.int32)
        return raw, host, (tuple(a.shape[0] for a in ints), tuple(sizes), n_int, fl.shape[0])

    def meta_views(self, rb: RaggedBatch, devbuf: Tensor, layout):
        lens, sizes, n_int, n_fl = layout
        d, off = {}, 0
        for n, ln, s in zip(self.META_NAMES, lens, sizes):
            d[n] = devbuf[off:off + ln]; off += s
        fdev = devbuf[n_int:n_int + n_fl].view(F32)
        d['cond_times'], d['row_time'] = fdev[:rb.n_cond], fdev[rb.n_cond:]
        d['h2d_bytes'] = devbuf.numel() * 4
        d['_keep'] = devbuf
        d['_layout'] = layout
        return d

    def upload(self, rb: RaggedBatch):
        if rb.dev:
            return rb.dev
        raw, host, layout = self.stage_meta(rb)
        devbuf = host.to(self.device, non_blocking = True)
        POOL.give(raw)
        rb.dev = self.meta_views(rb, devbuf, layout)
        return rb.dev

    def rope_table(self, max_pos: int):
        n = _round_up(max_pos + 1, 1024)
        t = self.ws.get('rope_cs')
        if t is None or t.shape[0] < n:
            if t is not None and self.graph_pins is not None:
                self.graph_pins += [t, self.ws['rope_cs_t']]
            t = torch.empty(n, 32, 2, device = self.device, dtype = F32)
            tt = torch.empty(32, n, 2, device = self.device, dtype = F32)
            self.ops.rope_table(self.model.rotary_emb.freqs.detach().float().contiguous(), t, tt, n, 32)
            self.ws['rope_cs'], self.ws['rope_cs_t'] = t, tt
        return t

    def _ptr_array(self, tensors):
        arr = (ctypes.c_void_p * len(tensors))(*[t.data_ptr() for t in tensors])
        self._ptr_arrays.append(arr)
        if len(self._ptr_arrays) > 256:
            self._ptr_arrays = self._ptr_arrays[-64:]
        return ctypes.cast(arr, ctypes.c_void_p)

    def forward(self, rb: RaggedBatch, latents: list | None, eps: list | None, *, train: bool, want_logits = False, vlimit = 0,
                text_loss_weight = 1., flow_loss_weight = 1., modality_only = False, cache: KVCache | None = None, want_preds = None,
                vel_targets = None, vel_weight = 0., dropout = False, dropout_key = None):
        self.ensure_attached()
        self.pack_weights(force = train)
        o, D, HI, H, Ip, M = self.ops, self.D, self.HI, self.H, self.Ip, rb.M
        dv = self.upload(rb)
        nc, S = rb.n_cond, rb.S
        p_ff = self.model.transformer.ff_dropout_p(train, dropout)
        st = self.state = dict(rb = rb, train = train, layers = [], p_ff = p_ff, drop_key = self.dropout_key(dropout_key) if p_ff > 0. else None)
        pk = self.packed
        rope = self.rope_table(rb.max_rope_pos)
        cond_row = dv['cond_row'] if nc > 0 else None
        tag = 'T' if train else 'I'
        assert cache is None or not train, 'the kv cache is an inference-time structure'
        kv_rows = dv['kv_row'] if cache is not None else None
        M_kv = cache.rows if cache is not None else 0
        want_preds = want_logits if want_preds is None else want_preds

        if nc > 0:
            feats = self.buf('feats', (nc, self.Kt), BF16)
            o.time_features(dv['cond_times'], self.model.transformer.to_time_cond[0].weights, feats, nc, D // 2, self.Kt)
            cpre = self.buf('cpre', (nc, 4 * D), F32)
            o.gemm_store(feats, self.Kt, 0, pk['wt'], self.Kt, 0, nc, 4 * D, self.Kt, cpre, 4 * D, None, 0, self.P('transformer.to_time_cond.1.bias'), None, 1.0, 0, 1)
            cond = self.buf('cond', (nc, 4 * D), BF16)
            o.table_op(cpre, 4 * D, None, 0, None, 0, cond, 4 * D, nc, 4 * D, 1)
            tab = self.buf('tab', (nc, self.W * 3 * D), F32)
            o.gemm_store(cond, 4 * D, 0, pk['wfz'], 4 * D, 0, nc, self.W * 3 * D, 4 * D, tab, self.W * 3 * D, None, 0, pk['bfz'], None, 1.0, 0, 1)
            zg = self.buf('zg', (nc, self.W * D), F32)
            for w in range(self.W):
                o.table_op(tab[:, w * 3 * D + 2 * D:], self.W * 3 * D, None, 0, zg[:, w * D:], self.W * D, None, 0, nc, D, 0)
            st.update(feats = feats, cpre = cpre, cond = cond, tab = tab, zg = zg)
        tab_ld, zg_ld = self.W * 3 * D, self.W * D

        modtok = None
        if S > 0:
            modtok = self.buf('modtok', (S, D), F32)
            st['noised'], st['flow'] = [], []
            for t, (s0, s1) in enumerate(rb.type_rows):
                n = s1 - s0
                if n == 0:
                    st['noised'].append(None); st['flow'].append(None); continue
                dl, dlp = self.dls[t], self.dlp[t]
                x = latents[t]
                assert x.shape == (n, dl) and x.dtype == F32 and x.is_cuda, f'latents[{t}] must be a cuda fp32 [{n}, {dl}] tensor'
                noised = self.buf(f'noised{t}', (n, dlp), BF16)
                if dlp != dl:
                    noised[:, dl:].zero_()
                has_proj = f'latent_to_model_projs.{t}.weight' in self.named
                nf32 = None if has_proj else modtok[s0:s1]
                if eps is not None and eps[t] is not None:
                    flow = self.buf(f'flow{t}', (n, dl), F32)
                    o.flow_noise(x, eps[t], dv['row_time'][s0:s1], noised, dlp, nf32, flow, n, dl)
                else:
                    flow = None
                    o.flow_noise(x, None, None, noised, dlp, None, None, n, dl)
                    if not has_proj:
                        modtok[s0:s1].copy_(x)
                if has_proj:
                    o.gemm_store(noised, dlp, 0, pk[f'wl2m{t}'], dlp, 0, n, D, dl, modtok[s0:s1], D, None, 0, self.P(f'latent_to_model_projs.{t}.bias'), None, 1.0, 0, 1)
                if self.posemb and self.posemb[t]:
                    nax = int(self.model.modality_num_dim[t])
                    coords = [dv[f'pos_c{a}'][s0:s1] for a in range(nax)]
                    tabs = posemb_tables(self._posemb_params(t, nax), rb.pos_max[t][:nax], self.device)
                    posemb_add(modtok[s0:s1], tabs, coords)
                    st.setdefault('posemb', {})[t] = (tabs, coords)
                st['noised'].append(noised); st['flow'].append(flow)
        x0 = self.buf(f'{tag}x0', (M, D), F32)
        x0b = self.buf(f'{tag}x0b', (M, D), BF16)
        o.embed_assemble(dv['text_id'], self.P('text_embed.weight'), modtok, dv['slot'] if S > 0 else None, x0, x0b, M, D)

        hid = [x0b if self.hid_bf16 else x0]
        skips = []
        x_in, x_in_b = x0, x0b
        n_tiles = int(rb.tile_q0.shape[0])
        for i in range(self.depth):
            L = {}
            pre = f'transformer.layers.{i}'
            lt = f'{tag}{i}' if train else 'I'
            layer = i + 1
            first_half = layer <= self.depth // 2
            if first_half:
                skips.append((i, x_in_b))
            has_skip = (not first_half) and f'{pre}.0.weight' in self.named
            if has_skip:
                src_i, skip_b = skips.pop()
                x_a = self.buf(f'{lt}xa', (M, D), F32)
                o.gemm_resid(x_in_b, D, skip_b, D, D, pk[f'wskip{i}'], 2 * D, M, D, 2 * D, None, x_in, x_a, None, None, None, None, 0, None)
                L.update(skip_src = src_i, skip_b = skip_b)
            else:
                x_a = x_in
            wA, wF = 2 * i, 2 * i + 1
            filmA = tab[:, wA * 3 * D:] if nc > 0 else None
            filmF = tab[:, wF * 3 * D:] if nc > 0 else None
            zgA = zg[:, wA * D:] if nc > 0 else None
            zgF = zg[:, wF * D:] if nc > 0 else None
            uA = self.buf(f'{lt}uA', (M, D), BF16); statsA = self.buf(f'{lt}sA', (M, 2), F32)
            o.adaln_fwd(x_a, cond_row, filmA, tab_ld, self.P(f'{pre}.1.layernorm_gamma'), uA, statsA, M, D)
            q = self.buf(f'{lt}q', (M, HI), BF16)
            if cache is not None:
                k, v = cache.k[i], cache.v[i]
            else:
                k = self.buf(f'{lt}k', (M, HI), BF16); v = self.buf(f'{lt}v0' if (self.vres and i == 0) else f'{lt}v', (M, HI), BF16)
            gates = self.buf(f'{lt}g', (M, H), F32); qk_inv = self.buf(f'{lt}qi', (M, 2 * H), F32)
            has_mix = self.vres and i > 0
            mixpre = self.buf(f'{lt}mix', (M, H), F32) if has_mix else None
            o.gemm_qkvg(uA, D, pk[f'qkvg{i}'], D, M, H, D, q, k, v, gates, qk_inv, self.P(f'{pre}.1.fn.q_norm.gamma'), self.P(f'{pre}.1.fn.k_norm.gamma'),
                        dv['rope_pos'], self.ws['rope_cs_t'], int(self.ws['rope_cs_t'].shape[1]), kv_rows, mixpre)
            if has_mix:
                v_first = cache.v[0] if cache is not None else st['layers'][0]['v']
                o.vmix_fwd(v, HI, kv_rows, v_first, HI, mixpre, self.P(f'{pre}.1.fn.to_learned_value_residual.0.bias'), M, H)
            v_att, att_gates = v, gates
            if self.laser:
                v_att = cache.vl[i] if cache is not None else self.buf(f'{lt}vl', (M, HI), BF16)
                o.laser_v_fwd(v, HI, kv_rows, v_att, HI, M, H, self.laser_clamp)
                att_gates = None
            att = self.buf(f'{lt}o', (M, HI), BF16); lse = self.buf(f'{lt}lse', (H, M), F32)
            o_l = self.buf(f'{lt}ol', (M, HI), BF16) if self.laser else att
            fp = self.fastp[i]
            if getattr(rb, 'single_row_tiles', False):
                o.attn_decode(q, k, v_att, HI, HI, HI, att_gates, H, dv['kv_limit'], dv['tile_q0'], dv['tile_kv0'], dv['tile_kvend'], n_tiles, o_l, HI, self.scale, self.softcap)
            else:
                o.attn_fwd_tc(q, k, v_att, HI, HI, HI, att_gates, H, dv['kv_limit'], dv['t2_q0'], dv['t2_qend'], dv['t2_kv0'], dv['t2_kvend'], int(rb.t2_q0.shape[0]),
                              o_l, HI, lse, M, M_kv, self.scale, self.softcap, fp)
                o.attn_fwd(q, k, v_att, HI, HI, HI, att_gates, H, dv['kv_limit'], dv['tile_q0'], dv['tile_qend'], dv['tile_kv0'], dv['tile_kvend'], n_tiles,
                           o_l, HI, lse, M, self.scale, self.softcap, fp)
            if self.laser:
                o.laser_out_fwd(o_l, gates, att, M, H)
            x_b = self.buf(f'{lt}xb', (M, D), F32); yA = self.buf(f'{lt}yA', (M, D), BF16) if train else None
            o.gemm_resid(att, HI, None, 0, 0, pk[f'wo{i}'], HI, M, D, HI, None, x_a, x_b, None, yA, cond_row, zgA, zg_ld, self.P(f'{pre}.1.layerscale'))
            uF = self.buf(f'{lt}uF', (M, D), BF16); statsF = self.buf(f'{lt}sF', (M, 2), F32)
            o.adaln_fwd(x_b, cond_row, filmF, tab_ld, self.P(f'{pre}.2.layernorm_gamma'), uF, statsF, M, D)
            vg = self.buf(f'{lt}vg', (M, 2 * Ip), BF16); h = self.buf(f'{lt}h', (M, Ip), BF16)
            if p_ff > 0.:
                o.gemm_geglu_drop(uF, D, pk[f'w1{i}'], D, pk[f'b1{i}'], M, 2 * Ip, D, vg, h, st['drop_key'], p_ff, i)
            else:
                o.gemm_geglu(uF, D, pk[f'w1{i}'], D, pk[f'b1{i}'], M, 2 * Ip, D, vg, h)
            yF = self.buf(f'{lt}yF', (M, D), BF16) if train else None
            if self.hid_bf16:
                x_c = self.buf(f'{tag}Hb{i + 1}', (M, D), BF16)
                o.gemm_resid(h, Ip, None, 0, 0, pk[f'w2{i}'], Ip, M, D, Ip, self.P(f'{pre}.2.fn.net.3.bias'), x_b, None, x_c, yF, cond_row, zgF, zg_ld,
                             self.P(f'{pre}.2.layerscale'))
            else:
                x_c = self.buf(f'{tag}H{i + 1}', (M, D), F32)
                o.gemm_resid(h, Ip, None, 0, 0, pk[f'w2{i}'], Ip, M, D, Ip, self.P(f'{pre}.2.fn.net.3.bias'), x_b, x_c, None, yF, cond_row, zgF, zg_ld,
                             self.P(f'{pre}.2.layerscale'))
            hid.append(x_c)
            xr = self.buf(f'{tag}xr{i}', (M, D), F32); xrb = self.buf(f'{tag}xrb{i}', (M, D), BF16)
            rlse = self.buf(f'{tag}rlse{i}', (M,), F32) if train else None
            (o.attn_residual_fwd_h16 if self.hid_bf16 else o.attn_residual_fwd)(self._ptr_array(hid), len(hid), self.P(f'{pre}.3.norm_keys.gamma'), self.P(f'{pre}.3.pseudo_queries'),
                                                                                 xr, xrb, rlse, M, D)
            L.update(xr = xr, rlse = rlse, mixpre = mixpre, o_l = o_l, v_att = v_att)
            L.update(x_a = x_a, uA = uA, statsA = statsA, q = q, k = k, v = v, gates = gates, qk_inv = qk_inv, att = att, lse = lse, yA = yA, x_b = x_b,
                     uF = uF, statsF = statsF, vg = vg, h = h, yF = yF, x_in = x_in, x_in_b = x_in_b, has_skip = has_skip, first_half = first_half)
            st['layers'].append(L)
            x_in, x_in_b = xr, xrb
        st['hid'] = hid
        st['x_last'] = x_in

        out = self.buf(f'{tag}out', (M, D), F32)
        outb = self.buf(f'{tag}outb', (M, D), BF16)
        omod = self.buf(f'{tag}omod', (max(S, 1), D), BF16)
        o.rmsnorm_fwd(x_in, self.P('transformer.norm.gamma'), out, outb, dv['slot'] if S > 0 else None, omod if S > 0 else None, M, D)
        if self.clean and S > 0:
            o.clean_flow_fwd(out, dv['row_token'], modtok, dv['cond_times'], dv['cond_row'], self.clean_eps, omod, S, D)
        st.update(out = out, outb = outb, omod = omod)
        res = dict(embed = out)

        if want_logits or train:
            logits = self.buf(f'{tag}logits', (M, self.Vp), F32)
            o.gemm_store(outb, D, 0, pk['wvocab'], D, 0, M, self.V, D, logits, self.Vp, None, 0, None, None, 1.0, 0, 1)
            res['logits'] = logits
            st['logits'] = logits
        preds = []
        if S > 0 and (train or want_preds):
            for t, (s0, s1) in enumerate(rb.type_rows):
                n = s1 - s0
                if n == 0:
                    preds.append(None); continue
                dl = self.dls[t]
                pred = self.buf(f'{tag}pred{t}', (n, dl), F32)
                o.gemm_store(omod[s0:s1], D, 0, pk[f'wm2l{t}'], D, 0, n, dl, D, pred, dl, None, 0, None, None, 1.0, 0, 1)
                preds.append(pred)
            res['preds'] = preds
        if train:
            T = float(rb.total_tokens)
            acc = self.buf('lossacc', (2 + len(self.dls),), torch.float64)
            acc.zero_()
            nvalid = self.buf('nvalid', (1,), I32); nvalid.zero_()
            dlog = self.buf('dlogits', (M, self.Vp), BF16)
            if modality_only:
                dlog.zero_()
            else:
                gs = (text_loss_weight / T) if vlimit == 0 else 1.0 / max(rb.n_valid, 1)
                o.ce_fwd_bwd(logits, self.Vp, dv['label'], self.V, vlimit, gs, dlog, self.Vp, acc[0:1], nvalid, M)
            st['dlogits'] = dlog
            st['dpred'] = []
            flow_terms = []
            vel_terms = {}
            for t, (s0, s1) in enumerate(rb.type_rows):
                n = s1 - s0
                if n == 0 or st['flow'][t] is None:
                    st['dpred'].append(None); flow_terms.append(None); continue
                dl, dlp = self.dls[t], self.dlp[t]
                wt = 1.0 if modality_only else rb.n_type_tokens[t] / T
                dpred = self.buf(f'dpred{t}', (n, dlp), BF16)
                if dlp != dl:
                    dpred[:, dl:].zero_()
                ga = 2.0 * flow_loss_weight * wt / (n * dl)
                if vel_targets is not None and vel_targets[t] is not None and vel_weight != 0.:
                    e = vel_targets[t]
                    assert e.shape == (n, dl) and e.dtype == F32
                    gb = 2.0 * vel_weight * wt / (n * dl)
                    vacc = self.buf('velacc', (len(self.dls),), torch.float64)
                    if t == 0 or not vel_terms:
                        vacc.zero_()
                    o.mse_fwd_bwd(preds[t], dl, e, None, dlp, gb, vacc[t: t + 1], n, dl)
                    o.mse_fwd_bwd(preds[t], dl, st['flow'][t], None, dlp, ga, acc[1 + t: 2 + t], n, dl)
                    blend = self.buf(f'velblend{t}', (n, dl), F32)
                    blend.zero_()
                    o.axpy_f32(blend, st['flow'][t], ga / (ga + gb), n * dl)
                    o.axpy_f32(blend, e, gb / (ga + gb), n * dl)
                    scratch = self.buf('velscratch', (1,), torch.float64)
                    o.mse_fwd_bwd(preds[t], dl, blend, dpred, dlp, ga + gb, scratch, n, dl)
                    vel_terms[t] = (vacc[t] / (n * dl)).float()
                else:
                    o.mse_fwd_bwd(preds[t], dl, st['flow'][t], dpred, dlp, ga, acc[1 + t: 2 + t], n, dl)
                st['dpred'].append(dpred)
                flow_terms.append((acc[1 + t] / (n * dl)).float() )
            text = (acc[0] / nvalid[0].clamp(min = 1)).float()
            flows = torch.stack([f if f is not None else torch.zeros((), device = self.device) for f in flow_terms]) if flow_terms else torch.zeros(0, device = self.device)
            if vlimit:
                total = text.clone()
            elif modality_only:
                total = flows.sum()
            else:
                total = (acc[0] / T).float() * text_loss_weight
                for t, f in enumerate(flow_terms):
                    if f is not None:
                        total = total + f * (rb.n_type_tokens[t] / T) * flow_loss_weight
                for t, f in vel_terms.items():
                    total = total + f * (rb.n_type_tokens[t] / T) * vel_weight
            vel = [vel_terms.get(t, torch.zeros((), device = self.device)) for t in range(len(self.dls))] if vel_terms else None
            res.update(loss_acc = acc, n_valid = nvalid, total = total, text = text, flows = flows, vel = vel)
        return res

    def dropout_key(self, src = None, out: Tensor | None = None) -> Tensor:
        if torch.is_tensor(src):
            assert src.dtype == I32 and src.numel() == 2 and src.device == self.device, 'a dropout key tensor is int32 [2] on the engine device'
            return src
        key = out if out is not None else self.buf('drop_key', (2,), I32)
        if src is None:
            key.random_(-2 ** 31, 2 ** 31)
        else:
            key.copy_(torch.from_numpy(np.array(src, dtype = np.uint32).view(np.int32)))
        return key

    def _prepare_grads(self):
        missing = [(n, p) for n, p in self.named.items() if p.grad is None or p.grad.data_ptr() != self.gflat.data_ptr() + 4 * self.offs[n]]
        if not missing:
            return
        if len(missing) == len(self.named):
            self.gflat.zero_()
        for n, p in missing:
            gv = self.G(n)
            if len(missing) != len(self.named):
                gv.zero_()
            if p.grad is not None:
                gv.copy_(p.grad)
            p.grad = gv

    def backward(self, gscale = None, bucket_cb = None):
        st = self.state
        assert st['train'], 'backward() needs a train forward'
        self._prepare_grads()
        self._grads_clean = False
        self._dirty = True
        if gscale is not None:
            gs = gscale.detach().float().reshape(1)
            self.ops.scale_bf16(st['dlogits'], gs, st['dlogits'].numel())
            for dp in st['dpred']:
                if dp is not None:
                    self.ops.scale_bf16(dp, gs, dp.numel())
        rb, dv = st['rb'], st['rb'].dev
        o, D, HI, H, Ip, M, inner = self.ops, self.D, self.HI, self.H, self.Ip, st['rb'].M, self.inner
        pk, nc, S = self.packed, rb.n_cond, rb.S
        cond_row = dv['cond_row'] if nc > 0 else None
        tab_ld, zg_ld = self.W * 3 * D, self.W * D
        ks = max(1, min(64, M // 2048))
        sms = torch.cuda.get_device_properties(self.device).multi_processor_count
        def ksplit(n_out, n_in, K = M):
            tiles = ((n_out + 127) // 128) * ((n_in + 255) // 256 if (n_in % 256 == 0 or n_in >= 1024) else (n_in + 127) // 128)
            best, best_eff = 1, 0.0
            for s in range(1, 65):
                if K // s < 1024 and s > 1:
                    break
                items = tiles * s
                eff = items / (-(-items // sms) * sms)
                if eff > best_eff + 0.02 or (abs(eff - best_eff) <= 0.02 and s <= ks and s > best):
                    best, best_eff = s, eff
            return best
        def wgrad(dy, ld_dy, n_out, act, ld_act, n_in, gname, K = M):
            o.gemm_store(dy, ld_dy, 1, act, ld_act, 1, n_out, n_in, K, self.G(gname), n_in, None, 0, None, None, 1.0, 1, ksplit(n_out, n_in, K))

        dlog = st['dlogits']
        d_out = self.buf('d_out', (M, D), F32)
        o.gemm_store(dlog, self.Vp, 0, pk['wvocab'], D, 1, M, D, self.V, d_out, D, None, 0, None, None, 1.0, 0, 1)
        wgrad(dlog, self.Vp, self.V, st['outb'], D, D, 'to_text_logits.weight')
        if S > 0:
            dmod = self.buf('dmod', (S, D), F32)
            any_flow = False
            for t, (s0, s1) in enumerate(rb.type_rows):
                n = s1 - s0
                dp = st['dpred'][t] if n else None
                if dp is None:
                    if n:
                        dmod[s0:s1].zero_()
                    continue
                any_flow = True
                dl, dlp = self.dls[t], self.dlp[t]
                o.gemm_store(dp, dlp, 0, pk[f'wm2l{t}'], D, 1, n, D, dl, dmod[s0:s1], D, None, 0, None, None, 1.0, 0, 1)
                wgrad(dp, dlp, dl, st['omod'][s0:s1], D, D, f'model_to_latent_projs.{t}.weight', K = n)
            dneg = None
            if any_flow and self.clean:
                dneg = self.buf('dmod_neg', (S, D), F32)
                o.clean_flow_bwd(dmod, dneg, dv['row_token'], dv['cond_times'], dv['cond_row'], self.clean_eps, S, D)
            if any_flow:
                o.scatter_add_rows(d_out, dmod, dv['row_token'], S, D)
        g = self.buf('gx', (M, D), F32)
        o.rmsnorm_bwd(d_out, st['x_last'], self.P('transformer.norm.gamma'), g, self.G('transformer.norm.gamma'), M, D)

        hid = st['hid']
        dH = [self.buf(f'dH{l}', (M, D), F32) for l in range(self.depth + 1)]
        dskip = {}
        if nc > 0:
            dtab = self.buf('dtab', (nc, self.W * 3 * D), F32); dtab.zero_()
            dzg = self.buf('dzg', (nc, self.W * D), F32); dzg.zero_()
        dy = self.buf('dy', (M, D), BF16)
        du = self.buf('du', (M, D), F32)
        arws = self.buf('attn_res_ws', (int(o.lib.tfx_attn_residual_bwd_workspace_floats(M, D)),), F32)
        sc_stride = (self.depth + 2) * 3
        arsc = self.buf('attn_res_sc', (self.depth, M, self.depth + 2, 3), F32) if self.ares_deferred else None
        dxs = {}
        for i in reversed(range(self.depth)):
            L = st['layers'][i]
            pre = f'transformer.layers.{i}'
            lm = self.layer_maps[i]
            wA, wF = 2 * i, 2 * i + 1
            if self.ares_deferred:
                dxs[i] = g
                later = list(range(i + 1, self.depth))
                gam = [self.P(f'transformer.layers.{j}.3.norm_keys.gamma') for j in [i] + later]
                pqs = [self.P(f'transformer.layers.{j}.3.pseudo_queries') for j in [i] + later]
                o.attn_residual_bwd2(self._ptr_array(hid[:i + 2]), i + 2, 1, self._ptr_array(gam), self._ptr_array(pqs), self._ptr_array([dxs[j] for j in later] or [g]),
                                     self._ptr_array([arsc[j][0, i + 1] for j in later] or [g]), len(later), g, L['xr'], L['rlse'], dH[i + 1], arsc[i], sc_stride,
                                     self.G(f'{pre}.3.norm_keys.gamma'), self.G(f'{pre}.3.pseudo_queries'), arws, M, D)
            else:
              (o.attn_residual_bwd_h16 if self.hid_bf16 else o.attn_residual_bwd)(self._ptr_array(hid[:i + 2]), self._ptr_array(dH[:i + 2]), i + 2, self.P(f'{pre}.3.norm_keys.gamma'), self.P(f'{pre}.3.pseudo_queries'),
                                g, L['xr'], L['rlse'], self.G(f'{pre}.3.norm_keys.gamma'), self.G(f'{pre}.3.pseudo_queries'), arws, M, D, 1 if i == self.depth - 1 else 0)
            gx = dH[i + 1]
            o.resid_bwd(gx, L['yF'], cond_row, st['zg'][:, wF * D:] if nc > 0 else None, zg_ld, self.P(f'{pre}.2.layerscale'), dy,
                        dzg[:, wF * D:] if nc > 0 else None, zg_ld, self.G(f'{pre}.2.layerscale'), self.G(f'{pre}.2.fn.net.3.bias'), M, D)
            dh = self.buf('dh', (M, Ip), BF16)
            o.gemm_store(dy, D, 0, pk[f'w2{i}'], Ip, 1, M, Ip, D, None, 0, dh, Ip, None, None, 1.0, 0, 1)
            o.gemm_store(dy, D, 1, L['h'], Ip, 1, D, inner, M, self.gflat, 0, None, 0, None, lm['w2_rows'], 1.0, 1, ksplit(D, inner))
            dvg = self.buf('dvg', (M, 2 * Ip), BF16)
            rpb = self.ops.lib.tfx_geglu_bwd_rows_per_block()
            nblk = (M + rpb - 1) // rpb
            part = self.buf('geglu_part', (nblk, 2 * Ip), F32)
            if st['p_ff'] > 0.:
                o.geglu_bwd_drop(dh, L['vg'], dvg, M, Ip, None, None, part, st['drop_key'], st['p_ff'], i)
            else:
                o.geglu_bwd(dh, L['vg'], dvg, M, Ip, None, None, part)
            o.colsum_f32(part, 2 * Ip, nblk, 2 * Ip, lm['b1_cols'], self.gflat)
            o.gemm_store(dvg, 2 * Ip, 0, pk[f'w1{i}'], D, 1, M, D, 2 * Ip, du, D, None, 0, None, None, 1.0, 0, 1)
            o.gemm_store(dvg, 2 * Ip, 1, L['uF'], D, 1, 2 * Ip, D, M, self.gflat, 0, None, 0, None, lm['w1_rows'], 1.0, 1, ksplit(2 * Ip, D))
            o.adaln_bwd(du, L['x_b'], L['statsF'], cond_row, st['tab'][:, wF * 3 * D:] if nc > 0 else None, tab_ld, self.P(f'{pre}.2.layernorm_gamma'), gx,
                        dtab[:, wF * 3 * D:] if nc > 0 else None, tab_ld, self.G(f'{pre}.2.layernorm_gamma'), M, D)
            o.resid_bwd(gx, L['yA'], cond_row, st['zg'][:, wA * D:] if nc > 0 else None, zg_ld, self.P(f'{pre}.1.layerscale'), dy,
                        dzg[:, wA * D:] if nc > 0 else None, zg_ld, self.G(f'{pre}.1.layerscale'), None, M, D)
            dog = self.buf('dog', (M, HI), BF16)
            o.gemm_store(dy, D, 0, pk[f'wo{i}'], HI, 1, M, HI, D, None, 0, dog, HI, None, None, 1.0, 0, 1)
            wgrad(dy, D, D, L['att'], HI, HI, f'{pre}.1.fn.to_out.1.weight')
            dop = self.buf('dop', (M, HI), BF16); dsum_hm = self.buf('dsum_hm', (H, M), F32); dsum_mh = self.buf('dsum_mh', (M, H), F32)
            dq = self.buf('dq', (M, HI), F32); dk = self.buf('dk', (M, HI), F32)
            if self.laser:
                o.laser_bwd_prep(dog, L['o_l'], L['gates'], dop, dsum_hm, dsum_mh, dq, M, H)
            else:
                o.attn_bwd_prep(dog, L['att'], L['gates'], dop, dsum_hm, dsum_mh, dq, M, H)
            dqkvg = self.buf('dqkvg', (M, self.NQ), BF16)
            if i == self.depth - 1:
                dqkvg[:, 3 * HI + H:].zero_()
            fp = self.fastp[i]
            o.attn_bwd_tc(L['q'], L['k'], L['v_att'], dop, HI, HI, HI, HI, L['lse'], dsum_hm, dv['kv_limit'], dv['k2_kv0'], dv['k2_kvend'], dv['k2_q0'], dv['k2_qend'],
                          dv['k2_order'], int(rb.k2_kv0.shape[0]), dq, dk, dqkvg[:, 2 * HI:], self.NQ, M, H, self.scale, self.softcap, fp)
            o.attn_bwd(L['q'], L['k'], L['v_att'], dop, HI, HI, HI, HI, L['lse'], dsum_hm, dv['kv_limit'], dv['kt_kv0'], dv['kt_kvend'], dv['kt_q0'], dv['kt_qend'],
                       int(rb.kt_kv0.shape[0]), dq, dk, dqkvg[:, 2 * HI:], self.NQ, M, H, self.scale, self.softcap, fp)
            dv_cols = dqkvg[:, 2 * HI:]
            if self.laser:
                o.laser_v_bwd(dv_cols, self.NQ, L['v'], HI, M, H, self.laser_clamp)
            if self.vres:
                dv0 = self.buf('dv_first', (M, HI), F32)
                if i == self.depth - 1:
                    dv0.zero_()
                if i > 0:
                    o.vmix_bwd(dv_cols, self.NQ, L['v'], HI, st['layers'][0]['v'], HI, L['mixpre'], self.P(f'{pre}.1.fn.to_learned_value_residual.0.bias'), dv0,
                               dqkvg[:, 3 * HI + H:], self.NQ, M, H)
                    o.colsum_bf16(dqkvg[:, 3 * HI + H:], self.NQ, M, H, None, self.G(f'{pre}.1.fn.to_learned_value_residual.0.bias'))
                else:
                    dqkvg[:, 3 * HI + H:3 * HI + 2 * H].zero_()
                    o.add_f32_into_bf16(dv_cols, self.NQ, dv0, HI, M, HI)
            o.qk_bwd_pack(dq, dk, L['q'], L['k'], L['qk_inv'], self.P(f'{pre}.1.fn.q_norm.gamma'), self.P(f'{pre}.1.fn.k_norm.gamma'), dv['rope_pos'],
                          self.ws['rope_cs'], L['gates'], dsum_mh, dqkvg, self.NQ, self.G(f'{pre}.1.fn.q_norm.gamma'), self.G(f'{pre}.1.fn.k_norm.gamma'), M, H)
            o.gemm_store(dqkvg, self.NQ, 0, pk[f'qkvg{i}'], D, 1, M, D, self.NQ, du, D, None, 0, None, None, 1.0, 0, 1)
            o.gemm_store(dqkvg, self.NQ, 1, L['uA'], D, 1, self.NQ, D, M, self.gflat, 0, None, 0, None, lm['qkvg_rows'], 1.0, 1, ksplit(self.NQ, D))
            o.adaln_bwd(du, L['x_a'], L['statsA'], cond_row, st['tab'][:, wA * 3 * D:] if nc > 0 else None, tab_ld, self.P(f'{pre}.1.layernorm_gamma'), gx,
                        dtab[:, wA * 3 * D:] if nc > 0 else None, tab_ld, self.G(f'{pre}.1.layernorm_gamma'), M, D)
            if L['has_skip']:
                o.resid_bwd(gx, None, None, None, 0, None, dy, None, 0, None, None, M, D)
                wsk = pk[f'wskip{i}']
                gw = self.G(f'{pre}.0.weight')
                o.gemm_store(dy, D, 1, L['x_in_b'], D, 1, D, D, M, gw, 2 * D, None, 0, None, None, 1.0, 1, ksplit(D, D))
                o.gemm_store(dy, D, 1, L['skip_b'], D, 1, D, D, M, gw.view(-1)[D:], 2 * D, None, 0, None, None, 1.0, 1, ksplit(D, D))
                src = L['skip_src']
                assert src not in dskip
                dskip[src] = self.buf(f'dskip{src}', (M, D), F32)
                o.gemm_store(dy, D, 0, wsk[:, D:], 2 * D, 1, M, D, D, dskip[src], D, None, 0, None, None, 1.0, 0, 1)
                o.gemm_store(dy, D, 0, wsk, 2 * D, 1, M, D, D, gx, D, None, 0, None, None, 1.0, 1, 1)
            if i in dskip:
                o.axpy_f32(gx, dskip[i], 1.0, M * D)
            g = gx
            if bucket_cb is not None:
                bucket_cb(i)
        if self.ares_deferred:
            allj = list(range(self.depth))
            gam = [self.P(f'transformer.layers.{j}.3.norm_keys.gamma') for j in [0] + allj]
            pqs = [self.P(f'transformer.layers.{j}.3.pseudo_queries') for j in [0] + allj]
            o.attn_residual_bwd2(self._ptr_array(hid[:1]), 1, 0, self._ptr_array(gam), self._ptr_array(pqs), self._ptr_array([dxs[j] for j in allj]),
                                 self._ptr_array([arsc[j][0, 0] for j in allj]), len(allj), None, None, None, dH[0], None, sc_stride, None, None, None, M, D)
        o.axpy_f32(g, dH[0], 1.0, M * D)
        dmodtok = self.buf('dmodtok', (max(S, 1), D), BF16)
        o.embed_bwd(g, dv['text_id'], dv['slot'] if S > 0 else None, self.G('text_embed.weight'), dmodtok if S > 0 else None, M, D)
        if S > 0:
            if self.clean and dneg is not None:
                o.add_f32_into_bf16(dmodtok, D, dneg, D, S, D)
            for t, (tabs, coords) in st.get('posemb', {}).items():
                s0, s1 = rb.type_rows[t]
                nax = len(tabs)
                posemb_backward(dmodtok[s0:s1].float(), tabs, coords, self._posemb_params(t, nax), self._posemb_params(t, nax, grads = True))
            for t, (s0, s1) in enumerate(rb.type_rows):
                n = s1 - s0
                if n == 0 or f'latent_to_model_projs.{t}.weight' not in self.named:
                    continue
                dl, dlp = self.dls[t], self.dlp[t]
                o.gemm_store(dmodtok[s0:s1], D, 1, st['noised'][t], dlp, 1, D, dl, n, self.G(f'latent_to_model_projs.{t}.weight'), dl, None, 0, None, None, 1.0, 1,
                             max(1, min(ks, n // 128)))
                o.colsum_bf16(dmodtok[s0:s1], D, n, D, None, self.G(f'latent_to_model_projs.{t}.bias'))
        if nc > 0:
            W3 = self.W * 3 * D
            for w in range(self.W):
                o.table_op(dzg[:, w * D:], zg_ld, st['zg'][:, w * D:], zg_ld, dtab[:, w * 3 * D + 2 * D:], W3, None, 0, nc, D, 2)
            dtabb = self.buf('dtabb', (nc, W3), BF16)
            o.cast_bf16(dtab, dtabb, nc * W3)
            dcond = self.buf('dcond', (nc, 4 * D), F32)
            o.gemm_store(dtabb, W3, 0, pk['wfz'], 4 * D, 1, nc, 4 * D, W3, dcond, 4 * D, None, 0, None, None, 1.0, 0, 1)
            o.gemm_store(dtabb, W3, 1, st['cond'], 4 * D, 1, W3, 4 * D, nc, self.gflat, 0, None, 0, None, self.fz_rows, 1.0, 1, 1)
            bsum = self.buf('bsum', (W3,), F32); bsum.zero_()
            o.colsum_f32(dtab, W3, nc, W3, None, bsum)
            self.gflat.index_add_(0, self.fz_bias_idx, bsum)
            dcpre = self.buf('dcpre', (nc, 4 * D), BF16)
            o.table_op(dcond, 4 * D, st['cpre'], 4 * D, None, 0, dcpre, 4 * D, nc, 4 * D, 3)
            o.gemm_store(dcpre, 4 * D, 1, st['feats'], self.Kt, 1, 4 * D, D + 1, nc, self.gflat, 0, None, 0, None, self.wt_rows, 1.0, 1, 1)
            o.colsum_bf16(dcpre, 4 * D, nc, 4 * D, None, self.G('transformer.to_time_cond.1.bias'))

    def new_cache(self, n_slabs: int, cap: int) -> KVCache:
        self.ensure_attached()
        return KVCache(self, n_slabs, cap)

    def text_decoder(self, cache, S, **kw):
        from .decode import TextDecoder
        return TextDecoder(self, cache, S, **kw)

    def ode_solve(self, cache, rb, y, **kw):
        from .decode import ode_solve
        return ode_solve(self, cache, rb, y, **kw)

    def zero_grad(self):
        if not getattr(self, '_grads_clean', False):
            self.gflat.zero_()
        self._grads_clean = False

    def clip_grad_norm_(self, max_norm: float, pre_scale: float = 1.0):
        ss = self.buf('gnorm_ss', (1,), torch.float64)
        ss.zero_()
        n = self.gflat.numel()
        self.ops.grad_sumsq(self.gflat, n, ss)
        self.ops.clip_by_norm(self.gflat, n, ss, float(max_norm), float(pre_scale))
        return ss.sqrt() * pre_scale

    def ema_update(self, decay: float):
        if getattr(self, 'ema_flat', None) is None or self.ema_flat.numel() != self.flat.numel():
            self.ema_flat = self.flat.clone()
            return
        self.ops.ema_update(self.ema_flat, self.flat, self.flat.numel(), float(decay))

    def ema_state_dict(self):
        assert getattr(self, 'ema_flat', None) is not None, 'no EMA update has run yet'
        return {n: self.ema_flat[o:o + self.named[n].numel()].view(self.named[n].shape) for n, o in self.offs.items()}

    def adam_step(self, lr = 1e-3, betas = (0.9, 0.999), eps = 1e-8, weight_decay = 0., decoupled = False, grad_scale = 1.0, zero_grads = False, device_step = False):
        if self.exp_avg is None:
            self.exp_avg = torch.zeros_like(self.flat); self.exp_avg_sq = torch.zeros_like(self.flat)
        self.opt_step += 1
        step_dev = None
        if device_step:
            assert getattr(self, 'opt_step_dev', None) is not None, 'device_step needs engine.opt_step_dev (int32 [1] on the device)'
            step_dev = self.opt_step_dev
        self.ops.adam_step(self.flat, self.gflat, self.exp_avg, self.exp_avg_sq, self.flat.numel(), lr, betas[0], betas[1], eps, weight_decay, int(decoupled),
                           self.opt_step, grad_scale, int(zero_grads), step_dev)
        self._grads_clean = bool(zero_grads)
        self._dirty = True
```

transfusion_pytorch_b200/modality_processing.py:

```python
from __future__ import annotations

import math
from dataclasses import dataclass, field
from typing import Callable

import numpy as np
import torch
from torch import Tensor, is_tensor

ModalitySample = list

ATT_TILE = 64


def is_int_tensor(t) -> bool:
    return is_tensor(t) and t.dtype in (torch.int, torch.long)


@dataclass
class ModalityInstance:
    batch_index: int
    modality_type: int
    offset: int
    length: int
    axial_shape: tuple
    row0: int
    cond_row: int
    token0: int = -1


@dataclass
class RaggedBatch:
    B: int
    M: int
    seq_lens: np.ndarray
    cu: np.ndarray
    full_lens: np.ndarray
    text_id: np.ndarray
    label: np.ndarray
    kv_limit: np.ndarray
    rope_pos: np.ndarray
    cond_row: np.ndarray
    slot: np.ndarray
    n_cond: int
    cond_times: np.ndarray
    n_types: int
    type_rows: list
    row_token: np.ndarray
    row_time: np.ndarray
    latents: list
    instances: list
    modality_positions: list
    total_tokens: int
    n_type_tokens: list
    tile_q0: np.ndarray = None
    tile_qend: np.ndarray = None
    tile_kv0: np.ndarray = None
    tile_kvend: np.ndarray = None
    kt_kv0: np.ndarray = None
    kt_kvend: np.ndarray = None
    kt_q0: np.ndarray = None
    kt_qend: np.ndarray = None
    t2_q0: np.ndarray = None
    t2_qend: np.ndarray = None
    t2_kv0: np.ndarray = None
    t2_kvend: np.ndarray = None
    k2_kv0: np.ndarray = None
    k2_kvend: np.ndarray = None
    k2_q0: np.ndarray = None
    k2_qend: np.ndarray = None
    k2_order: np.ndarray = None
    pos_c0: np.ndarray = None
    pos_c1: np.ndarray = None
    pos_c2: np.ndarray = None
    pos_max: tuple = None
    kv_row: np.ndarray = None
    single_row_tiles: bool = False
    max_rope_pos: int = 0
    has_labels: bool = False
    n_valid: int = 0
    dev: dict = field(default_factory = dict)

    @property
    def S(self) -> int:
        return int(self.row_token.shape[0])


def _meta_ids(model, axial: tuple, modality_type: int):
    cache = model.__dict__.setdefault('_meta_id_cache', {})
    key = (axial, modality_type)
    hit = cache.get(key)
    if hit is None:
        chars = [ord(c) + model.meta_id + 1 for c in ','.join(map(str, axial))]
        hit = cache[key] = (np.asarray([model.meta_id] + chars + [model.som_ids[modality_type]], dtype = np.int64), np.asarray([model.eom_ids[modality_type]], dtype = np.int64))
    return hit


_NEG = np.full(4096, -1, dtype = np.int64)


def _neg_ids(n: int):
    global _NEG
    if n > _NEG.shape[0]:
        _NEG = np.full(max(n, 2 * _NEG.shape[0]), -1, dtype = np.int64)
    return _NEG[:n]


ATT_GROUP_TOKENS = 8192


def build_tiles(rb: RaggedBatch, qfirst: np.ndarray) -> None:
    cu, lens = rb.cu.astype(np.int64), rb.seq_lens.astype(np.int64)
    kv_limit = np.asarray(rb.kv_limit)
    qfirst = np.asarray(qfirst)
    for T, pre_q, pre_k in ((ATT_TILE, 'tile', 'kt'), (2 * ATT_TILE, 't2', 'k2')):
        ntiles = (lens + T - 1) // T
        total = int(ntiles.sum())
        if total == 0:
            z = np.zeros(0, dtype = np.int32)
            for name in (f'{pre_q}_q0', f'{pre_q}_qend', f'{pre_q}_kv0', f'{pre_q}_kvend', f'{pre_k}_kv0', f'{pre_k}_kvend', f'{pre_k}_q0', f'{pre_k}_qend'):
                setattr(rb, name, z)
            rb.k2_order = z
            continue
        seq = np.repeat(np.arange(rb.B), ntiles)
        first = np.cumsum(ntiles) - ntiles
        tin = np.arange(total) - first[seq]
        s = cu[:-1][seq]
        q0 = s + tin * T
        qe = np.minimum(q0 + T, s + lens[seq])
        kve = np.maximum.reduceat(kv_limit, q0) + 1
        kq0 = s + ((qfirst[q0] - s) // T) * T
        as32 = lambda a: np.ascontiguousarray(a, dtype = np.int32)
        for name, arr in ((f'{pre_q}_q0', q0), (f'{pre_q}_qend', qe), (f'{pre_q}_kv0', s), (f'{pre_q}_kvend', kve),
                          (f'{pre_k}_kv0', q0), (f'{pre_k}_kvend', qe), (f'{pre_k}_q0', kq0), (f'{pre_k}_qend', s + lens[seq])):
            setattr(rb, name, as32(arr))
        if pre_k == 'k2':
            group = s // ATT_GROUP_TOKENS if rb.M >= 12 * ATT_GROUP_TOKENS else np.zeros_like(s)
            rb.k2_order = as32(np.lexsort((-(s + lens[seq] - kq0), group)))


def pack_batch(
    modalities: list,
    times,
    model,
    *,
    return_loss: bool,
    return_embed: bool,
    need_axial_pos_emb: bool = False,
) -> RaggedBatch:
    B = len(modalities)
    n_types = model.num_modalities
    times_np = None
    if times is not None:
        times_np = times.detach().float().cpu().numpy() if is_tensor(times) else np.asarray(times, dtype = np.float32)

    pieces, piece_inst, sample_piece0, full_lens = [], [], [], []
    instances: list[ModalityInstance] = []
    latents = [[] for _ in range(n_types)]
    type_counts = [0] * n_types
    modality_positions = []
    cond_times = []
    dim_latents, channel_first, num_dim = model.dim_latents, model.channel_first_latent, model.modality_num_dim
    n_time_cols = times_np.shape[1] if times_np is not None else 0
    for b, sample in enumerate(modalities):
        offset, mi, positions = 0, 0, []
        sample_piece0.append(len(pieces))
        for item in sample:
            if isinstance(item, tuple):
                mtype, mt = item[0], item[1]
            elif item.is_floating_point():
                mtype, mt = 0, item
            else:
                assert item.dtype in (torch.int, torch.long) and item.ndim <= 1, 'text must be a 0-d or 1-d int tensor'
                arr = item.numpy() if (item.device.type == 'cpu' and not item.requires_grad) else item.detach().cpu().numpy()
                if arr.ndim != 1:
                    arr = arr.reshape(-1)
                pieces.append(arr); piece_inst.append(-1); offset += arr.shape[0]
                continue
            assert 0 <= mtype < n_types, f'received a modality index that is out of range. only {n_types} modalities specified'
            dl = dim_latents[mtype]
            cf = channel_first[mtype]
            assert mt.shape[0 if cf else -1] == dl, f'mismatch for modality latent dimension - expected {dl} but received {mt.shape[0 if cf else -1]} - modality shape is {tuple(mt.shape)}, perhaps you need to set `channel_first_latent` to the correct value'
            nd = num_dim[mtype]
            assert nd is None or nd == mt.ndim - 1, f'mismatch for modality number of dimensions - expected {nd} but received {mt.ndim - 1} {tuple(mt.shape)}'
            axial = tuple(mt.shape[1:]) if cf else tuple(mt.shape[:-1])
            length = axial[0] if len(axial) == 1 else math.prod(axial)
            flat = (mt.reshape(dl, length).t() if cf else (mt if mt.ndim == 2 else mt.reshape(length, dl)))
            pre = 0
            if not return_embed:
                meta, eom = _meta_ids(model, axial, mtype)
                pieces.append(meta); piece_inst.append(-1); pre = meta.shape[0]
            pieces.append(_neg_ids(length)); piece_inst.append(len(instances))
            if not return_embed:
                pieces.append(eom); piece_inst.append(-1)
            t_val = float(times_np[b, mi]) if n_time_cols > mi else 0.
            inst = ModalityInstance(b, mtype, offset + pre, length, axial, type_counts[mtype], len(cond_times))
            cond_times.append(t_val)
            type_counts[mtype] += length
            latents[mtype].append(flat)
            instances.append(inst); positions.append((mtype, offset + pre, length))
            offset += pre + length + (0 if return_embed else 1)
            mi += 1
        full_lens.append(offset); modality_positions.append(positions)
    sample_piece0.append(len(pieces))

    full_lens = np.asarray(full_lens, dtype = np.int64)
    drop = 1 if return_loss else 0
    seq_lens = np.maximum(full_lens - drop, 0)
    cu = np.zeros(B + 1, dtype = np.int64); np.cumsum(seq_lens, out = cu[1:])
    M = int(cu[-1])

    type_base = np.concatenate([[0], np.cumsum(type_counts)]).astype(np.int64)
    S = int(type_base[-1])

    P = len(pieces)
    plen = np.fromiter((p.shape[0] for p in pieces), dtype = np.int64, count = P)
    pinst = np.asarray(piece_inst, dtype = np.int64)
    fed_pieces, lab_pieces = pieces, None
    if drop and P:
        fed_pieces, lab_pieces, plen = list(pieces), list(pieces), plen.copy()
        for b in range(B):
            lo, hi = sample_piece0[b], sample_piece0[b + 1]
            j = hi - 1
            while j >= lo and plen[j] == 0: j -= 1
            if j >= lo:
                fed_pieces[j] = fed_pieces[j][:-1]; plen[j] -= 1
            j = lo
            while j < hi and lab_pieces[j].shape[0] == 0: j += 1
            if j < hi:
                lab_pieces[j] = lab_pieces[j][1:]
    ar = np.arange(M, dtype = np.int64)
    pstart = np.cumsum(plen) - plen
    is_mod = np.repeat(pinst >= 0, plen)
    qfirst64 = np.where(is_mod, np.repeat(pstart, plen), ar)
    kv_limit = np.where(is_mod, np.repeat(pstart + plen - 1, plen), ar).astype(np.int32)
    qfirst = qfirst64.astype(np.int32)
    n_type_tokens = [0] * n_types
    row_token = np.full(S, -1, dtype = np.int32); row_time = np.zeros(S, dtype = np.float32)
    cond_row = np.full(M, -1, dtype = np.int32); slot = np.full(M, -1, dtype = np.int32)
    if instances:
        ni = len(instances)
        il = np.fromiter((i.length for i in instances), dtype = np.int64, count = ni)
        ity = np.fromiter((i.modality_type for i in instances), dtype = np.int64, count = ni)
        ir0 = type_base[ity] + np.fromiter((i.row0 for i in instances), dtype = np.int64, count = ni)
        ic = np.fromiter((i.cond_row for i in instances), dtype = np.int64, count = ni)
        ct = np.asarray(cond_times, dtype = np.float32)
        ipiece = np.nonzero(pinst >= 0)[0]
        cnt, tok0 = plen[ipiece], pstart[ipiece]
        for inst, c, t0 in zip(instances, cnt.tolist(), tok0.tolist()):
            if c:
                inst.token0 = t0
        pc = np.full(P, -1, dtype = np.int64); pc[ipiece] = ic
        pr = np.zeros(P, dtype = np.int64); pr[ipiece] = ir0 - tok0
        cond_row = np.repeat(pc, plen).astype(np.int32)
        slot = np.where(is_mod, np.repeat(pr, plen) + ar, -1).astype(np.int32)
        order = np.argsort(ir0, kind = 'stable')
        il_s, r0_s = il[order], ir0[order]
        rr = np.arange(S, dtype = np.int64) - np.repeat(r0_s, il_s)
        row_token = np.where(rr < np.repeat(cnt[order], il_s), np.repeat(tok0[order], il_s) + rr, -1).astype(np.int32)
        row_time = np.repeat(ct[ic[order]], il_s)
        n_type_tokens = [int(c) for c in np.bincount(ity, weights = cnt, minlength = n_types)]
    text_id = np.zeros(M, dtype = np.int32); label = np.full(M, -1, dtype = np.int32); rope_pos = np.zeros(M, dtype = np.int32)
    max_rope = 0
    if M:
        ids_fed = np.concatenate(fed_pieces)
        assert ids_fed.shape[0] == M
        text_id = np.maximum(ids_fed, 0).astype(np.int32)
        seq_of = np.repeat(np.arange(B), seq_lens)
        seq_start = cu[:-1][seq_of]
        ce = np.cumsum(is_mod & (ar != qfirst64))
        before = np.where(seq_start > 0, ce[np.maximum(seq_start - 1, 0)], 0)
        pos = (ar - seq_start) - (ce - before)
        rope_pos = pos.astype(np.int32)
        max_rope = int(pos.max())
        if return_loss:
            lab = np.concatenate(lab_pieces).astype(np.int64)
            assert lab.shape[0] == M
            lab[is_mod] = -1
            lab[lab == model.null_text_id] = -1
            label = lab.astype(np.int32)

    rb = RaggedBatch(
        B = B, M = M, seq_lens = seq_lens, cu = cu, full_lens = full_lens, text_id = text_id, label = label, kv_limit = kv_limit,
        rope_pos = rope_pos, cond_row = cond_row, slot = slot, n_cond = len(cond_times),
        cond_times = np.asarray(cond_times, dtype = np.float32), n_types = n_types,
        type_rows = [(int(type_base[t]), int(type_base[t + 1])) for t in range(n_types)], row_token = row_token, row_time = row_time,
        latents = latents, instances = instances, modality_positions = modality_positions,
        total_tokens = int(full_lens.sum()), n_type_tokens = n_type_tokens, max_rope_pos = max_rope, has_labels = return_loss)
    rb.n_valid = int((label >= 0).sum())
    add_pos = getattr(model, 'add_pos_emb', None)
    if add_pos is not None and any(add_pos) and instances:
        coords = [np.full(S, -1, dtype = np.int32) for _ in range(3)]
        pmax = [None] * n_types
        for inst in instances:
            t = inst.modality_type
            if not add_pos[t]:
                continue
            ax = tuple(int(a) for a in inst.axial_shape)
            assert len(ax) <= 3, 'axial positional embeddings are implemented for up to 3 axes'
            r0 = int(type_base[t]) + inst.row0
            for a, c in enumerate(np.unravel_index(np.arange(inst.length), ax)):
                coords[a][r0:r0 + inst.length] = c
            pmax[t] = ax if pmax[t] is None else tuple(max(x, y) for x, y in zip(pmax[t], ax))
        rb.pos_c0, rb.pos_c1, rb.pos_c2 = coords
        rb.pos_max = tuple(None if m is None else tuple((x + 7) // 8 * 8 for x in m) for m in pmax)
    build_tiles(rb, qfirst)
    return rb


def pack_incremental(samples: list, times, model, *, slab: np.ndarray, base_len: np.ndarray, rope_base: np.ndarray, cap: int) -> RaggedBatch:
    rb = pack_batch(samples, times, model, return_loss = False, return_embed = True)
    B, M = rb.B, rb.M
    slab, base_len, rope_base = (np.asarray(a, dtype = np.int64) for a in (slab, base_len, rope_base))
    assert slab.shape == base_len.shape == rope_base.shape == (B,)
    assert ((base_len + rb.seq_lens) <= cap).all(), 'kv cache slab overflow: a sample needs more rows than the slab capacity'
    off = slab * cap + base_len - rb.cu[:-1]
    seq = np.repeat(np.arange(B), rb.seq_lens)
    rb.kv_row = (np.arange(M, dtype = np.int64) + off[seq]).astype(np.int32)
    rb.kv_limit = (rb.kv_limit.astype(np.int64) + off[seq]).astype(np.int32)
    rb.rope_pos = (rb.rope_pos.astype(np.int64) + rope_base[seq]).astype(np.int32)
    rb.max_rope_pos = int(rb.rope_pos.max()) if M else 0
    for pre in ('tile', 't2'):
        q0 = getattr(rb, f'{pre}_q0')
        if q0.shape[0] == 0:
            continue
        ts = np.searchsorted(rb.cu, q0, side = 'right') - 1
        setattr(rb, f'{pre}_kv0', (slab[ts] * cap).astype(np.int32))
        setattr(rb, f'{pre}_kvend', (getattr(rb, f'{pre}_kvend').astype(np.int64) + off[ts]).astype(np.int32))
    rb.single_row_tiles = bool(M > 0 and (rb.seq_lens <= 1).all())
    return rb


def pack_text_only(text: Tensor, *, return_loss: bool, pos_offset: int = 0) -> RaggedBatch:
    t = text.detach().cpu().numpy().astype(np.int64)
    B, L = t.shape
    n = L - 1 if return_loss else L
    M = B * n
    cu = np.arange(B + 1, dtype = np.int64) * n
    tid = t[:, :n].reshape(-1)
    label = np.full(M, -1, dtype = np.int32)
    if return_loss:
        label = t[:, 1:].reshape(-1).astype(np.int32)
    rb = RaggedBatch(
        B = B, M = M, seq_lens = np.full(B, n, dtype = np.int64), cu = cu, full_lens = np.full(B, L, dtype = np.int64),
        text_id = np.where(tid < 0, 0, tid).astype(np.int32), label = label, kv_limit = np.arange(M, dtype = np.int32),
        rope_pos = (np.tile(np.arange(n, dtype = np.int32), B) + pos_offset).astype(np.int32), cond_row = np.full(M, -1, dtype = np.int32),
        slot = np.full(M, -1, dtype = np.int32), n_cond = 0, cond_times = np.zeros(0, dtype = np.float32), n_types = 0, type_rows = [],
        row_token = np.zeros(0, dtype = np.int32), row_time = np.zeros(0, dtype = np.float32), latents = [], instances = [],
        modality_positions = [[] for _ in range(B)], total_tokens = B * L, n_type_tokens = [], max_rope_pos = n - 1 + pos_offset,
        has_labels = return_loss)
    rb.n_valid = int((label >= 0).sum())
    build_tiles(rb, np.arange(M, dtype = np.int32))
    return rb


def _strategy(name):
    def fn(modalities, times, model, *, need_axial_pos_emb, return_loss, return_embed):
        return pack_batch(modalities, times, model, return_loss = return_loss, return_embed = return_embed, need_axial_pos_emb = need_axial_pos_emb)
    fn.__name__ = f'process_modality_batch_{name}'
    return fn

PROCESSING_STRATEGIES: dict[str, Callable] = {name: _strategy(name) for name in ('naive', 'grouped', 'flat', 'hybrid', 'auto')}
DEFAULT_PROCESSING_STRATEGY = 'auto'


def get_processing_strategy(name: str):
    assert name in PROCESSING_STRATEGIES, f'unknown modality processing strategy `{name}`, available: {list(PROCESSING_STRATEGIES)}'
    return PROCESSING_STRATEGIES[name]
```

Measured before the change: 1.204 million.

## Shrink attention backward CTA to one warpgroup and run two CTAs per SM

The tensor-core attention backward kernel drops from two consumer warpgroups (128 keys per CTA) to one warpgroup handling 64-key chunks, looping over key chunks inside the CTA. Shared memory is cut (fewer stages, single dS buffer) so two CTAs can co-reside per SM. The engine switches to 64-token KV tiles with their own ordering array, and dQ reduction uses double-buffered staging with partial bulk waits. The goal is better SM occupancy and load balance on short ragged sequences, at the cost of reloading Q/dO once per key chunk and more block-wide syncs.

Measured after the change: 1.220 million, median of 6. 1.4% higher.

```diff
diff --git a/include/tfx_b200.h b/include/tfx_b200.h
--- a/include/tfx_b200.h
+++ b/include/tfx_b200.h
@@ -47,6 +47,7 @@
                     const float* lse, const float* dsum_hm, const int* kv_limit, const int* kt_kv0, const int* kt_kvend, const int* kt_q0, const int* kt_qend,
                     const int* kt_order ,
                     int n_kv_tiles, float* dq, float* dk, void* dv, long long ld_dv, int M, int H, float scale, float softcap, const float* fast_params, void* stream);
+int tfx_attn_bwd_tc_ctas_per_sm(void);
 int tfx_qk_bwd_pack(const float* dq, const float* dk, const void* q_bf16, const void* k_bf16, const float* qk_inv, const float* q_gamma, const float* k_gamma,
                     const int* rope_pos, const float* rope_cs, const float* gates, const float* dsum_mh, void* dqkvg_bf16, long long out_ld,
                     float* dq_gamma, float* dk_gamma, int M, int H, void* stream);
diff --git a/transfusion_pytorch_b200/_lib.py b/transfusion_pytorch_b200/_lib.py
--- a/transfusion_pytorch_b200/_lib.py
+++ b/transfusion_pytorch_b200/_lib.py
@@ -74,7 +74,7 @@
     'tfx_add_f32_into_bf16': [VP, LL, VP, LL, I, I, VP],
 }
 
-EXPORTED = ['tfx_last_error', 'tfx_version', 'tfx_geglu_bwd_rows_per_block', 'tfx_attn_residual_bwd_workspace_floats'] + list(SIGNATURES)
+EXPORTED = ['tfx_last_error', 'tfx_version', 'tfx_geglu_bwd_rows_per_block', 'tfx_attn_residual_bwd_workspace_floats', 'tfx_attn_bwd_tc_ctas_per_sm'] + list(SIGNATURES)
 
 
 class TfxError(RuntimeError):
@@ -103,6 +103,8 @@
     lib.tfx_geglu_bwd_rows_per_block.argtypes = []
     lib.tfx_attn_residual_bwd_workspace_floats.restype = c_longlong
     lib.tfx_attn_residual_bwd_workspace_floats.argtypes = [c_int, c_int]
+    lib.tfx_attn_bwd_tc_ctas_per_sm.restype = c_int
+    lib.tfx_attn_bwd_tc_ctas_per_sm.argtypes = []
     for name, argtypes in SIGNATURES.items():
         fn = getattr(lib, name)
         fn.argtypes = argtypes
diff --git a/transfusion_pytorch_b200/csrc/attention_sm90.cu b/transfusion_pytorch_b200/csrc/attention_sm90.cu
--- a/transfusion_pytorch_b200/csrc/attention_sm90.cu
+++ b/transfusion_pytorch_b200/csrc/attention_sm90.cu
@@ -168,19 +168,19 @@
 }
 
 
-constexpr int FB_BQ = 64;
-constexpr int FB_THREADS = 256;
-constexpr int FB_STAGES = 4;
+constexpr int FB_BQ = 64, FB_BK = 64;
+constexpr int FB_THREADS = 128;
+constexpr int FB_STAGES = 3;
 constexpr int FB_STAGE = 16384;
-constexpr int FB_RING = 32768;
+constexpr int FB_RING = 16384;
 constexpr int FB_ROW_BOX = FB_BQ + 4;
 constexpr int FB_ROW_SLOT = 384, FB_ROWS_STAGE = 3 * FB_ROW_SLOT;
 constexpr int FB_ROWS = FB_RING + FB_STAGES * FB_STAGE;
 constexpr int FB_DS = FB_ROWS + ((FB_STAGES * FB_ROWS_STAGE + 1023) & ~1023);
-constexpr int FB_DQ = FB_DS + 2 * 16384;
+constexpr int FB_DQ = FB_DS + 8192;
 constexpr int FB_BAR = FB_DQ + 2 * 16384;
 constexpr int FB_SMEM = FB_BAR + 256 + 1024 ;
-constexpr int FB_BAR_DS_FULL = 1, FB_BAR_DS_EMPTY = 3, FB_BAR_DQ = 5;
+static_assert(2 * (FB_SMEM + 1024) <= 228 * 1024, "attn_bwd_tc: two CTAs must fit one SM");
 
 template <bool MASKED>
 __device__ __forceinline__ void bwd_p(float (&sacc)[32], uint32_t (&pf)[4][4], const int* sLim, const float* sLse, int key_a, int key_b, int qvalid,
@@ -211,7 +211,7 @@
   }
 }
 
-__global__ void __launch_bounds__(FB_THREADS, 1)
+__global__ void __launch_bounds__(FB_THREADS, 2)
 attn_bwd_tc_k(const __grid_constant__ CUtensorMap tmQ, const __grid_constant__ CUtensorMap tmK, const __grid_constant__ CUtensorMap tmV,
               const __grid_constant__ CUtensorMap tmDO, const __grid_constant__ CUtensorMap tmLim, const __grid_constant__ CUtensorMap tmLse,
               const __grid_constant__ CUtensorMap tmD, const __grid_constant__ CUtensorMap tmDQ,
@@ -220,10 +220,11 @@
               const float* __restrict__ fast) {
   if (fast[0] == 0.f) return;
   extern __shared__ uint8_t fb_smem_raw[];
-  uint8_t* smem = reinterpret_cast<uint8_t*>((reinterpret_cast<uintptr_t>(fb_smem_raw) + 1023) & ~uintptr_t(1023));
+  uint8_t* smem = fb_smem_raw + ((1024u - (smem_u32(fb_smem_raw) & 1023u)) & 1023u);
   uint8_t* sK = smem;
-  uint8_t* sV = smem + 16384;
+  uint8_t* sV = smem + 8192;
   uint8_t* sDS = smem + FB_DS;
+  uint8_t* sDQ = smem + FB_DQ;
   uint64_t* bars = reinterpret_cast<uint64_t*>(smem + FB_BAR);
   uint64_t *full = bars, *empty = bars + FB_STAGES, *kv_full = bars + 2 * FB_STAGES;
 
@@ -233,11 +234,13 @@
   const int head = idx - tt * H;
   const int kv0 = kt_kv0[tile], kv_end = kt_kvend[tile], q_begin = kt_q0[tile], q_end = kt_qend[tile];
   const int n_q = (q_end - q_begin + FB_BQ - 1) / FB_BQ;
+  const int n_kc = (kv_end - kv0 + FB_BK - 1) / FB_BK;
+  const int n_steps = n_kc * n_q;
   const int tid = threadIdx.x, warp = tid >> 5, lane = tid & 31;
 
   if (tid == 0) {
     tma_prefetch_desc(&tmQ); tma_prefetch_desc(&tmK); tma_prefetch_desc(&tmV); tma_prefetch_desc(&tmDO);
-    for (int s = 0; s < FB_STAGES; ++s) { mbar_init(&full[s], 1); mbar_init(&empty[s], 8); }
+    for (int s = 0; s < FB_STAGES; ++s) { mbar_init(&full[s], 1); mbar_init(&empty[s], 4); }
     mbar_init(kv_full, 1);
     mbar_fence_init();
   }
@@ -245,7 +248,7 @@
 
   auto load_step = [&](int j) {
     const int sl = j % FB_STAGES;
-    const int qb = q_begin + j * FB_BQ;
+    const int qb = q_begin + (j % n_q) * FB_BQ;
     uint8_t* st = smem + FB_RING + sl * FB_STAGE;
     uint8_t* rows = smem + FB_ROWS + sl * FB_ROWS_STAGE;
     mbar_expect_tx(&full[sl], FB_STAGE + 3 * FB_ROW_BOX * 4);
@@ -255,88 +258,90 @@
     tma_load_1d(&tmLse, &full[sl], rows + FB_ROW_SLOT, (head * M + qb) & ~3);
     tma_load_1d(&tmD, &full[sl], rows + 2 * FB_ROW_SLOT, (head * M + qb) & ~3);
   };
+  auto load_kv = [&](int c) {
+    mbar_expect_tx(kv_full, 16384);
+    tma_load_2d(&tmK, kv_full, sK, head * 64, kv0 + c * FB_BK);
+    tma_load_2d(&tmV, kv_full, sV, head * 64, kv0 + c * FB_BK);
+  };
   if (tid == 0) {
-    mbar_expect_tx(kv_full, 32768);
-    tma_load_2d(&tmK, kv_full, sK, head * 64, kv0);
-    tma_load_2d(&tmV, kv_full, sV, head * 64, kv0);
-    for (int j = 0; j < FB_STAGES && j < n_q; ++j) load_step(j);
-  }
-  const int cwg = warp >> 2, w4 = warp & 3, g = lane >> 2, t = lane & 3;
-  const bool leader = (tid & 127) == 0;
+    load_kv(0);
+    for (int j = 0; j < FB_STAGES && j < n_steps; ++j) load_step(j);
+  }
+  const int g = lane >> 2, t = lane & 3;
+  const bool leader = tid == 0;
   const FaPoly poly(scale, cap);
   const float KL = cap * 1.4426950408889634f;
   const float oms_c = -scale / (KL * KL);
-  const int key_a = kv0 + cwg * 64 + w4 * 16 + g, key_b = key_a + 8;
-  const int warp_key_last = kv0 + cwg * 64 + w4 * 16 + 15;
-  float dvacc[32], dkacc[32];
-#pragma unroll
-  for (int i = 0; i < 32; ++i) { dvacc[i] = 0.f; dkacc[i] = 0.f; }
-  const uint32_t aK = smem_u32(sK) + cwg * 8192, aV = smem_u32(sV) + cwg * 8192, aKall = smem_u32(sK);
-  const int ds_row0 = cwg * 64 + w4 * 16 + g;
-  uint8_t* sDQ = smem + FB_DQ + cwg * 16384;
-  mbar_wait(kv_full, 0);
-
-  int s = 0; uint32_t phase = 0;
-  for (int i = 0; i < n_q; ++i) {
-    const int b = i & 1;
-    const int qb = q_begin + i * FB_BQ;
-    mbar_wait(&full[s], phase);
-    const uint32_t aQ = smem_u32(smem + FB_RING + s * FB_STAGE), aDO = aQ + 8192;
-    const int* sLim = reinterpret_cast<const int*>(smem + FB_ROWS + s * FB_ROWS_STAGE) + (qb & 3);
-    const float* sLse = reinterpret_cast<const float*>(smem + FB_ROWS + s * FB_ROWS_STAGE + FB_ROW_SLOT) + ((head * M + qb) & 3);
-    const float* sD = reinterpret_cast<const float*>(smem + FB_ROWS + s * FB_ROWS_STAGE + 2 * FB_ROW_SLOT) + ((head * M + qb) & 3);
-    float sacc[32], pacc[32];
-    wgmma_fence();
-#pragma unroll
-    for (int k = 0; k < 4; ++k) wgmma_m64n64_ss<0, 0>(sacc, wgmma_desc_sw128(aK + k * 32, 16, 1024), wgmma_desc_sw128(aQ + k * 32, 16, 1024), k > 0 ? 1u : 0u);
-    wgmma_commit();
-#pragma unroll
-    for (int k = 0; k < 4; ++k) wgmma_m64n64_ss<0, 0>(pacc, wgmma_desc_sw128(aV + k * 32, 16, 1024), wgmma_desc_sw128(aDO + k * 32, 16, 1024), k > 0 ? 1u : 0u);
-    wgmma_commit();
-    if (tid == 0 && i >= 2 && i - 2 + FB_STAGES < n_q) {
-      mbar_wait(&empty[(i - 2) % FB_STAGES], ((i - 2) / FB_STAGES) & 1);
-      load_step(i - 2 + FB_STAGES);
-    }
-    const int qvalid = q_end - qb;
-    const bool full_vis = qvalid >= FB_BQ && warp_key_last <= __reduce_min_sync(0xffffffffu, min(sLim[lane], sLim[lane + 32]));
-    wgmma_wait<1>();
-    wgmma_reg_fence(sacc);
-    uint32_t pf[4][4], dsf[4][4];
-    if (full_vis) bwd_p<false>(sacc, pf, sLim, sLse, key_a, key_b, qvalid, poly, oms_c, scale, t);
-    else bwd_p<true>(sacc, pf, sLim, sLse, key_a, key_b, qvalid, poly, oms_c, scale, t);
-    wgmma_wait<0>();
-    wgmma_reg_fence(pacc);
-#pragma unroll
-    for (int n8 = 0; n8 < 8; ++n8) {
-      const float d0 = sD[n8 * 8 + 2 * t], d1 = sD[n8 * 8 + 2 * t + 1];
-      dsf[n8 >> 1][(n8 & 1) * 2] = pack_bf16(sacc[4 * n8] * (pacc[4 * n8] - d0), sacc[4 * n8 + 1] * (pacc[4 * n8 + 1] - d1));
-      dsf[n8 >> 1][(n8 & 1) * 2 + 1] = pack_bf16(sacc[4 * n8 + 2] * (pacc[4 * n8 + 2] - d0), sacc[4 * n8 + 3] * (pacc[4 * n8 + 3] - d1));
-    }
-    uint8_t* dsb = sDS + b * 16384;
-    if (cwg != b && i >= 2) named_bar_sync(FB_BAR_DS_EMPTY + b, 256);
-#pragma unroll
-    for (int n8 = 0; n8 < 8; ++n8) {
-      const int r0 = ds_row0, r1 = ds_row0 + 8;
-      *reinterpret_cast<uint32_t*>(dsb + r0 * 128 + ((n8 ^ (r0 & 7)) << 4) + t * 4) = dsf[n8 >> 1][(n8 & 1) * 2];
-      *reinterpret_cast<uint32_t*>(dsb + r1 * 128 + ((n8 ^ (r1 & 7)) << 4) + t * 4) = dsf[n8 >> 1][(n8 & 1) * 2 + 1];
-    }
-    fence_proxy_async_smem();
-    if (cwg == b) named_bar_sync(FB_BAR_DS_FULL + b, 256);
-    else named_bar_arrive(FB_BAR_DS_FULL + b, 256);
-    wgmma_reg_fence(dvacc);
-    wgmma_reg_fence(dkacc);
-    wgmma_fence();
-#pragma unroll
-    for (int kk = 0; kk < 4; ++kk) wgmma_m64n64_rs<1>(dvacc, pf[kk], wgmma_desc_sw128(aDO + kk * 2048, 8192, 1024), 1u);
-#pragma unroll
-    for (int kk = 0; kk < 4; ++kk) wgmma_m64n64_rs<1>(dkacc, dsf[kk], wgmma_desc_sw128(aQ + kk * 2048, 8192, 1024), 1u);
-    wgmma_commit();
-    if (cwg == b) {
+  const uint32_t aK = smem_u32(sK), aV = smem_u32(sV), aDS = smem_u32(sDS);
+  const int ds_r0 = warp * 16 + g, ds_r1 = ds_r0 + 8;
+
+  int s = 0, step = 0; uint32_t phase = 0;
+  for (int c = 0; c < n_kc; ++c) {
+    if (c > 0) {
+      __syncthreads();
+      if (tid == 0) load_kv(c);
+    }
+    const int key_a = kv0 + c * FB_BK + warp * 16 + g, key_b = key_a + 8;
+    const int warp_key_last = kv0 + c * FB_BK + warp * 16 + 15;
+    float dvacc[32], dkacc[32];
+#pragma unroll
+    for (int i = 0; i < 32; ++i) { dvacc[i] = 0.f; dkacc[i] = 0.f; }
+    mbar_wait(kv_full, c & 1);
+
+    for (int i = 0; i < n_q; ++i, ++step) {
+      const int qb = q_begin + i * FB_BQ;
+      mbar_wait(&full[s], phase);
+      const uint32_t aQ = smem_u32(smem + FB_RING + s * FB_STAGE), aDO = aQ + 8192;
+      const int* sLim = reinterpret_cast<const int*>(smem + FB_ROWS + s * FB_ROWS_STAGE) + (qb & 3);
+      const float* sLse = reinterpret_cast<const float*>(smem + FB_ROWS + s * FB_ROWS_STAGE + FB_ROW_SLOT) + ((head * M + qb) & 3);
+      const float* sD = reinterpret_cast<const float*>(smem + FB_ROWS + s * FB_ROWS_STAGE + 2 * FB_ROW_SLOT) + ((head * M + qb) & 3);
+      float sacc[32], pacc[32];
+      wgmma_fence();
+#pragma unroll
+      for (int k = 0; k < 4; ++k) wgmma_m64n64_ss<0, 0>(sacc, wgmma_desc_sw128(aK + k * 32, 16, 1024), wgmma_desc_sw128(aQ + k * 32, 16, 1024), k > 0 ? 1u : 0u);
+      wgmma_commit();
+#pragma unroll
+      for (int k = 0; k < 4; ++k) wgmma_m64n64_ss<0, 0>(pacc, wgmma_desc_sw128(aV + k * 32, 16, 1024), wgmma_desc_sw128(aDO + k * 32, 16, 1024), k > 0 ? 1u : 0u);
+      wgmma_commit();
+      if (tid == 0 && step >= 1 && step - 1 + FB_STAGES < n_steps) {
+        mbar_wait(&empty[(step - 1) % FB_STAGES], ((step - 1) / FB_STAGES) & 1);
+        load_step(step - 1 + FB_STAGES);
+      }
+      const int qvalid = q_end - qb;
+      const bool full_vis = qvalid >= FB_BQ && warp_key_last <= __reduce_min_sync(0xffffffffu, min(sLim[lane], sLim[lane + 32]));
+      wgmma_wait<1>();
+      wgmma_reg_fence(sacc);
+      uint32_t pf[4][4], dsf[4][4];
+      if (full_vis) bwd_p<false>(sacc, pf, sLim, sLse, key_a, key_b, qvalid, poly, oms_c, scale, t);
+      else bwd_p<true>(sacc, pf, sLim, sLse, key_a, key_b, qvalid, poly, oms_c, scale, t);
+      wgmma_wait<0>();
+      wgmma_reg_fence(pacc);
+#pragma unroll
+      for (int n8 = 0; n8 < 8; ++n8) {
+        const float d0 = sD[n8 * 8 + 2 * t], d1 = sD[n8 * 8 + 2 * t + 1];
+        dsf[n8 >> 1][(n8 & 1) * 2] = pack_bf16(sacc[4 * n8] * (pacc[4 * n8] - d0), sacc[4 * n8 + 1] * (pacc[4 * n8 + 1] - d1));
+        dsf[n8 >> 1][(n8 & 1) * 2 + 1] = pack_bf16(sacc[4 * n8 + 2] * (pacc[4 * n8 + 2] - d0), sacc[4 * n8 + 3] * (pacc[4 * n8 + 3] - d1));
+      }
+      wgmma_reg_fence(dvacc);
+      wgmma_reg_fence(dkacc);
+      wgmma_fence();
+#pragma unroll
+      for (int kk = 0; kk < 4; ++kk) wgmma_m64n64_rs<1>(dvacc, pf[kk], wgmma_desc_sw128(aDO + kk * 2048, 8192, 1024), 1u);
+#pragma unroll
+      for (int kk = 0; kk < 4; ++kk) wgmma_m64n64_rs<1>(dkacc, dsf[kk], wgmma_desc_sw128(aQ + kk * 2048, 8192, 1024), 1u);
+      wgmma_commit();
+#pragma unroll
+      for (int n8 = 0; n8 < 8; ++n8) {
+        *reinterpret_cast<uint32_t*>(sDS + ds_r0 * 128 + ((n8 ^ (ds_r0 & 7)) << 4) + t * 4) = dsf[n8 >> 1][(n8 & 1) * 2];
+        *reinterpret_cast<uint32_t*>(sDS + ds_r1 * 128 + ((n8 ^ (ds_r1 & 7)) << 4) + t * 4) = dsf[n8 >> 1][(n8 & 1) * 2 + 1];
+      }
+      fence_proxy_async_smem();
+      if (leader) bulk_wait_read_1();
+      __syncthreads();
       float qacc[32];
-      const uint32_t aDS = smem_u32(dsb);
       wgmma_fence();
 #pragma unroll
-      for (int kk = 0; kk < 8; ++kk) wgmma_m64n64_ss<1, 1>(qacc, wgmma_desc_sw128(aDS + kk * 2048, 8192, 1024), wgmma_desc_sw128(aKall + kk * 2048, 8192, 1024), kk > 0 ? 1u : 0u);
+      for (int kk = 0; kk < 4; ++kk) wgmma_m64n64_ss<1, 1>(qacc, wgmma_desc_sw128(aDS + kk * 2048, 8192, 1024), wgmma_desc_sw128(aK + kk * 2048, 8192, 1024), kk > 0 ? 1u : 0u);
       wgmma_commit();
       wgmma_wait<0>();
       wgmma_reg_fence(dvacc);
@@ -344,44 +349,34 @@
       wgmma_reg_fence(qacc);
       __syncwarp();
       if (lane == 0) mbar_arrive(&empty[s]);
-      if (i + 2 < n_q) named_bar_arrive(FB_BAR_DS_EMPTY + b, 256);
-      if (leader) bulk_wait_read_all();
-      named_bar_sync(FB_BAR_DQ + cwg, 128);
-      const int r0 = w4 * 16 + g, r1 = r0 + 8;
 #pragma unroll
       for (int n8 = 0; n8 < 8; ++n8) {
         const int chunk = 2 * (n8 & 3) + (t >> 1), off = (n8 >> 2) * 8192 + (t & 1) * 8;
-        *reinterpret_cast<float2*>(sDQ + off + r0 * 128 + ((chunk ^ (r0 & 7)) << 4)) = make_float2(qacc[4 * n8], qacc[4 * n8 + 1]);
-        *reinterpret_cast<float2*>(sDQ + off + r1 * 128 + ((chunk ^ (r1 & 7)) << 4)) = make_float2(qacc[4 * n8 + 2], qacc[4 * n8 + 3]);
+        *reinterpret_cast<float2*>(sDQ + (step & 1) * 16384 + off + ds_r0 * 128 + ((chunk ^ (ds_r0 & 7)) << 4)) = make_float2(qacc[4 * n8], qacc[4 * n8 + 1]);
+        *reinterpret_cast<float2*>(sDQ + (step & 1) * 16384 + off + ds_r1 * 128 + ((chunk ^ (ds_r1 & 7)) << 4)) = make_float2(qacc[4 * n8 + 2], qacc[4 * n8 + 3]);
       }
       fence_proxy_async_smem();
-      named_bar_sync(FB_BAR_DQ + cwg, 128);
+      __syncthreads();
       if (leader) {
-        tma_reduce_add_2d(&tmDQ, sDQ, head * 64, qb);
-        tma_reduce_add_2d(&tmDQ, sDQ + 8192, head * 64 + 32, qb);
+        tma_reduce_add_2d(&tmDQ, sDQ + (step & 1) * 16384, head * 64, qb);
+        tma_reduce_add_2d(&tmDQ, sDQ + (step & 1) * 16384 + 8192, head * 64 + 32, qb);
         bulk_commit();
       }
-    } else {
-      wgmma_wait<0>();
-      wgmma_reg_fence(dvacc);
-      wgmma_reg_fence(dkacc);
-      __syncwarp();
-      if (lane == 0) mbar_arrive(&empty[s]);
-    }
-    if (++s == FB_STAGES) { s = 0; phase ^= 1; }
+      if (++s == FB_STAGES) { s = 0; phase ^= 1; }
+    }
+#pragma unroll
+    for (int n8 = 0; n8 < 8; ++n8) {
+      if (key_a < kv_end) {
+        *reinterpret_cast<float2*>(dk + (long long)key_a * H * 64 + head * 64 + n8 * 8 + 2 * t) = make_float2(dkacc[4 * n8], dkacc[4 * n8 + 1]);
+        *reinterpret_cast<uint32_t*>(dv + (long long)key_a * ld_dv + head * 64 + n8 * 8 + 2 * t) = pack_bf16(dvacc[4 * n8], dvacc[4 * n8 + 1]);
+      }
+      if (key_b < kv_end) {
+        *reinterpret_cast<float2*>(dk + (long long)key_b * H * 64 + head * 64 + n8 * 8 + 2 * t) = make_float2(dkacc[4 * n8 + 2], dkacc[4 * n8 + 3]);
+        *reinterpret_cast<uint32_t*>(dv + (long long)key_b * ld_dv + head * 64 + n8 * 8 + 2 * t) = pack_bf16(dvacc[4 * n8 + 2], dvacc[4 * n8 + 3]);
+      }
+    }
   }
   if (leader) bulk_wait_all();
-#pragma unroll
-  for (int n8 = 0; n8 < 8; ++n8) {
-    if (key_a < kv_end) {
-      *reinterpret_cast<float2*>(dk + (long long)key_a * H * 64 + head * 64 + n8 * 8 + 2 * t) = make_float2(dkacc[4 * n8], dkacc[4 * n8 + 1]);
-      *reinterpret_cast<uint32_t*>(dv + (long long)key_a * ld_dv + head * 64 + n8 * 8 + 2 * t) = pack_bf16(dvacc[4 * n8], dvacc[4 * n8 + 1]);
-    }
-    if (key_b < kv_end) {
-      *reinterpret_cast<float2*>(dk + (long long)key_b * H * 64 + head * 64 + n8 * 8 + 2 * t) = make_float2(dkacc[4 * n8 + 2], dkacc[4 * n8 + 3]);
-      *reinterpret_cast<uint32_t*>(dv + (long long)key_b * ld_dv + head * 64 + n8 * 8 + 2 * t) = pack_bf16(dvacc[4 * n8 + 2], dvacc[4 * n8 + 3]);
-    }
-  }
 }
 
 inline int make_tmap_rows(CUtensorMap* tm, CUtensorMapDataType type, const void* ptr, long long n) {
@@ -411,7 +406,19 @@
 using namespace tfx;
 #define ST(s) reinterpret_cast<cudaStream_t>(s)
 
+static bool bwd_tc_smem_attr() {
+  static bool attr_set = false;
+  if (!attr_set) attr_set = cudaFuncSetAttribute(attn_bwd_tc_k, cudaFuncAttributeMaxDynamicSharedMemorySize, FB_SMEM) == cudaSuccess;
+  return attr_set;
+}
+
 extern "C" {
+
+int tfx_attn_bwd_tc_ctas_per_sm(void) {
+  int n = 0;
+  if (!bwd_tc_smem_attr() || cudaOccupancyMaxActiveBlocksPerMultiprocessor(&n, attn_bwd_tc_k, FB_THREADS, FB_SMEM) != cudaSuccess) return -1;
+  return n;
+}
 
 int tfx_attn_fast_params(const float* q_gamma, const float* k_gamma, int dim_head, float scale, float softcap, float* params, void* stream) {
   TFX_REQUIRE(dim_head > 0 && softcap > 0.f, "attn_fast_params: bad arguments");
@@ -452,18 +459,14 @@
   TFX_REQUIRE(ld_q % 8 == 0 && ld_k % 8 == 0 && ld_v % 8 == 0 && ld_do % 8 == 0 && ld_dv % 8 == 0, "attn_bwd_tc: row pitches must be multiples of 8 bf16");
   CUtensorMap tq, tk, tv, tdo, tlim, tlse, td, tdq;
   int rc;
-  if ((rc = make_tmap_bf16(&tq, q, (long long)H * 64, M, ld_q, FB_BQ)) || (rc = make_tmap_bf16(&tk, k, (long long)H * 64, M, ld_k, FA_BN)) ||
-      (rc = make_tmap_bf16(&tv, v, (long long)H * 64, M, ld_v, FA_BN)) || (rc = make_tmap_bf16(&tdo, do_pre, (long long)H * 64, M, ld_do, FB_BQ)) ||
+  if ((rc = make_tmap_bf16(&tq, q, (long long)H * 64, M, ld_q, FB_BQ)) || (rc = make_tmap_bf16(&tk, k, (long long)H * 64, M, ld_k, FB_BK)) ||
+      (rc = make_tmap_bf16(&tv, v, (long long)H * 64, M, ld_v, FB_BK)) || (rc = make_tmap_bf16(&tdo, do_pre, (long long)H * 64, M, ld_do, FB_BQ)) ||
       (rc = make_tmap_rows(&tlim, CU_TENSOR_MAP_DATA_TYPE_INT32, kv_limit, M)) || (rc = make_tmap_rows(&tlse, CU_TENSOR_MAP_DATA_TYPE_FLOAT32, lse, (long long)H * M)) ||
       (rc = make_tmap_rows(&td, CU_TENSOR_MAP_DATA_TYPE_FLOAT32, dsum_hm, (long long)H * M)) || (rc = make_tmap_dq(&tdq, dq, M, H))) {
     set_error("attn_bwd_tc: cuTensorMapEncodeTiled failed (%d): kv_limit, lse, dsum and dq must be 16-byte aligned", rc);
     return rc;
   }
-  static bool attr_set = false;
-  if (!attr_set) {
-    if (cudaFuncSetAttribute(attn_bwd_tc_k, cudaFuncAttributeMaxDynamicSharedMemorySize, FB_SMEM) != cudaSuccess) { set_error("attn_bwd_tc: cannot raise dynamic smem"); return -2; }
-    attr_set = true;
-  }
+  if (!bwd_tc_smem_attr()) { set_error("attn_bwd_tc: cannot raise dynamic smem"); return -2; }
   attn_bwd_tc_k<<<n_kv_tiles * H, FB_THREADS, FB_SMEM, ST(stream)>>>(tq, tk, tv, tdo, tlim, tlse, td, tdq, kt_kv0, kt_kvend, kt_q0, kt_qend, kt_order, dk,
                                                                      (__nv_bfloat16*)dv, ld_dv, M, H, scale, softcap, fast_params);
   return check_launch("attn_bwd_tc");
diff --git a/transfusion_pytorch_b200/csrc/sm90_ptx.cuh b/transfusion_pytorch_b200/csrc/sm90_ptx.cuh
--- a/transfusion_pytorch_b200/csrc/sm90_ptx.cuh
+++ b/transfusion_pytorch_b200/csrc/sm90_ptx.cuh
@@ -69,6 +69,7 @@
 }
 __device__ __forceinline__ void bulk_commit() { asm volatile("cp.async.bulk.commit_group;" ::: "memory"); }
 __device__ __forceinline__ void bulk_wait_read_all() { asm volatile("cp.async.bulk.wait_group.read 0;" ::: "memory"); }
+__device__ __forceinline__ void bulk_wait_read_1() { asm volatile("cp.async.bulk.wait_group.read 1;" ::: "memory"); }
 __device__ __forceinline__ void bulk_wait_all() { asm volatile("cp.async.bulk.wait_group 0;" ::: "memory"); }
 __device__ __forceinline__ void tma_load_2d_multicast(const CUtensorMap* m, uint64_t* bar, void* smem, int c0, int c1, uint16_t mask) {
   asm volatile(
diff --git a/transfusion_pytorch_b200/engine.py b/transfusion_pytorch_b200/engine.py
--- a/transfusion_pytorch_b200/engine.py
+++ b/transfusion_pytorch_b200/engine.py
@@ -284,7 +284,7 @@
         self._dirty = False
 
     META_NAMES = ['text_id', 'label', 'kv_limit', 'rope_pos', 'cond_row', 'slot', 'tile_q0', 'tile_qend', 'tile_kv0', 'tile_kvend',
-                  'kt_kv0', 'kt_kvend', 'kt_q0', 'kt_qend', 'row_token', 't2_q0', 't2_qend', 't2_kv0', 't2_kvend', 'k2_kv0', 'k2_kvend', 'k2_q0', 'k2_qend', 'k2_order', 'kv_row', 'pos_c0', 'pos_c1', 'pos_c2']
+                  'kt_kv0', 'kt_kvend', 'kt_q0', 'kt_qend', 'kt_order', 'row_token', 't2_q0', 't2_qend', 't2_kv0', 't2_kvend', 'kv_row', 'pos_c0', 'pos_c1', 'pos_c2']
 
     def stage_meta(self, rb: RaggedBatch):
         ints = [getattr(rb, n) if getattr(rb, n) is not None else _EMPTY_I32 for n in self.META_NAMES]
@@ -733,8 +733,8 @@
             if i == self.depth - 1:
                 dqkvg[:, 3 * HI + H:].zero_()
             fp = self.fastp[i]
-            o.attn_bwd_tc(L['q'], L['k'], L['v_att'], dop, HI, HI, HI, HI, L['lse'], dsum_hm, dv['kv_limit'], dv['k2_kv0'], dv['k2_kvend'], dv['k2_q0'], dv['k2_qend'],
-                          dv['k2_order'], int(rb.k2_kv0.shape[0]), dq, dk, dqkvg[:, 2 * HI:], self.NQ, M, H, self.scale, self.softcap, fp)
+            o.attn_bwd_tc(L['q'], L['k'], L['v_att'], dop, HI, HI, HI, HI, L['lse'], dsum_hm, dv['kv_limit'], dv['kt_kv0'], dv['kt_kvend'], dv['kt_q0'], dv['kt_qend'],
+                          dv['kt_order'], int(rb.kt_kv0.shape[0]), dq, dk, dqkvg[:, 2 * HI:], self.NQ, M, H, self.scale, self.softcap, fp)
             o.attn_bwd(L['q'], L['k'], L['v_att'], dop, HI, HI, HI, HI, L['lse'], dsum_hm, dv['kv_limit'], dv['kt_kv0'], dv['kt_kvend'], dv['kt_q0'], dv['kt_qend'],
                        int(rb.kt_kv0.shape[0]), dq, dk, dqkvg[:, 2 * HI:], self.NQ, M, H, self.scale, self.softcap, fp)
             dv_cols = dqkvg[:, 2 * HI:]
diff --git a/transfusion_pytorch_b200/modality_processing.py b/transfusion_pytorch_b200/modality_processing.py
--- a/transfusion_pytorch_b200/modality_processing.py
+++ b/transfusion_pytorch_b200/modality_processing.py
@@ -61,6 +61,7 @@
     kt_kvend: np.ndarray = None
     kt_q0: np.ndarray = None
     kt_qend: np.ndarray = None
+    kt_order: np.ndarray = None
     t2_q0: np.ndarray = None
     t2_qend: np.ndarray = None
     t2_kv0: np.ndarray = None
@@ -120,7 +121,7 @@
             z = np.zeros(0, dtype = np.int32)
             for name in (f'{pre_q}_q0', f'{pre_q}_qend', f'{pre_q}_kv0', f'{pre_q}_kvend', f'{pre_k}_kv0', f'{pre_k}_kvend', f'{pre_k}_q0', f'{pre_k}_qend'):
                 setattr(rb, name, z)
-            rb.k2_order = z
+            setattr(rb, f'{pre_k}_order', z)
             continue
         seq = np.repeat(np.arange(rb.B), ntiles)
         first = np.cumsum(ntiles) - ntiles
@@ -134,9 +135,8 @@
         for name, arr in ((f'{pre_q}_q0', q0), (f'{pre_q}_qend', qe), (f'{pre_q}_kv0', s), (f'{pre_q}_kvend', kve),
                           (f'{pre_k}_kv0', q0), (f'{pre_k}_kvend', qe), (f'{pre_k}_q0', kq0), (f'{pre_k}_qend', s + lens[seq])):
             setattr(rb, name, as32(arr))
-        if pre_k == 'k2':
-            group = s // ATT_GROUP_TOKENS if rb.M >= 12 * ATT_GROUP_TOKENS else np.zeros_like(s)
-            rb.k2_order = as32(np.lexsort((-(s + lens[seq] - kq0), group)))
+        group = s // ATT_GROUP_TOKENS if rb.M >= 12 * ATT_GROUP_TOKENS else np.zeros_like(s)
+        setattr(rb, f'{pre_k}_order', as32(np.lexsort((-(s + lens[seq] - kq0), group))))
 
 
 def pack_batch(
```
